# kevslinger/DTQN

Measured on AMD Instinct MI355X. Metric: env-steps/sec + TD-updates/sec, DiscreteCarFlag-v0 ctx=50 b=32, 1/2/4/8 GPU, higher is better.
Workload: dtype f32; 1 GPU; DiscreteCarFlag-v0 shapes (BASELINE config 1): ctx=50, d_model=64, 8 heads, 2 layers, obs 3 f32, 3 actions, batch 32 per GPU, history 50, device replay 2500 x 200 steps; global_batch=32, parallelism=dp1, sampler=device

## Files before the change

### dtqn_amd/csrc/dtqn_api.cpp

```cpp
#include <hip/hip_runtime.h>

#include <cstdlib>

#include "dtqn_hip.h"
#include "dtqn_limits.h"

extern "C" const char* dtqn_build_info(void) {
#ifdef DTQN_BUILD_INFO
    return DTQN_BUILD_INFO;
#else
    return "dtqn_hip (unstamped build)";
#endif
}

static void* g_profile_buffer = nullptr;
extern "C" int dtqn_debug_set_profile_buffer(void* dev_buffer) {
    g_profile_buffer = dev_buffer;
    return DTQN_OK;
}
extern "C" void* dtqn_debug_profile_buffer(void) { return g_profile_buffer; }

static int policy_cus() {
    int dev = 0, n = 0;
    if (hipGetDevice(&dev) != hipSuccess || hipDeviceGetAttribute(&n, hipDeviceAttributeMultiprocessorCount, dev) != hipSuccess || n <= 0) return 256;
    return n;
}
extern "C" int dtqn_td_row_split(const DtqnNet* net, int batch) {
    if (!net || batch < 1) return 1;
    const int cus = policy_cus();
    const char* e = getenv("DTQN_ROW_SPLIT");
    if (e != nullptr && e[0] == '0') return 1;
    const bool covered = !net->tiled && net->lp == 64 && !net->identity &&
                         (net->d_model == 64 || (net->d_model == 128 && net->gate == DTQN_GATE_RES));
    if (!covered) return 1;
    if (e != nullptr && e[0] == '1') return 2;
    if (e != nullptr && e[0] == '4') return 4;
    if (3 * batch * 2 <= cus) return 4;
    if (net->d_model == 64) {
        if (batch * 4 <= cus) return 4;
        if (batch * 2 <= cus) return 2;
    }
    return 1;
}
extern "C" int dtqn_td_latency_mode(const DtqnNet* net, int batch) {
    if (dtqn_td_row_split(net, batch) < 2) return 0;
    const char* e = getenv("DTQN_ROW_SPLIT");
    if (e != nullptr && (e[0] == '1' || e[0] == '4')) return 1;
    return 3 * batch * 2 <= policy_cus() ? 1 : 0;
}
extern "C" int dtqn_td_prefers_tiled(const DtqnNet* net, int batch) {
    if (!net || batch < 1 || net->tiled) return 0;
    if (dtqn_ws_lite(net->tiled, net->d_model, net->head_dim, net->d_real))
        return dtqn_td_row_split(net, batch) == 4 && dtqn_td_latency_mode(net, batch) ? 0 : 1;
    const bool covered = net->d_model == 128 && net->gate == DTQN_GATE_RES && !net->identity && net->lp == 64 && net->dropout == 0.f &&
                         net->bag_size == 0;
    if (!covered) return 0;
    const char* e = getenv("DTQN_TRAIN_TILED");
    if (e != nullptr) return atoi(e) != 0 ? 1 : 0;
    return dtqn_td_row_split(net, batch) == 1 ? 1 : 0;
}
extern "C" int dtqn_td_xch_floats(const DtqnNet* net, int batch) {
    if (!net || batch < 1) return 0;
    return 3 * batch * net->num_layers * (3 * net->lp / 4) * 2 * net->d_model;
}
extern "C" int dtqn_td_xch_flags(const DtqnNet* net, int batch) {
    if (!net || batch < 1) return 0;
    return 3 * batch * net->num_layers * 6 + 16;
}

extern "C" int dtqn_td_update(const DtqnNet* net, const DtqnReplay* rp, const DtqnTd* td, void* stream) {
    int rc;
    if ((rc = dtqn_td_forward(net, rp, td, stream)) != DTQN_OK) return rc;
    if ((rc = dtqn_td_backward(net, rp, td, stream)) != DTQN_OK) return rc;
    if ((rc = dtqn_td_wgrad(net, td, stream)) != DTQN_OK) return rc;
    if ((rc = dtqn_td_reduce(net, td, stream)) != DTQN_OK) return rc;
    return dtqn_td_clip_adam(net, td, stream);
}

extern "C" int dtqn_td_gradients_pipelined(const DtqnNet* net, const DtqnReplay* rp, const DtqnTd* td, const DtqnTd* td_next, int have_target,
                                           int draw_step, void* stream) {
    int rc;
    if (draw_step < 0) return DTQN_ERR_ARG;
    if ((rc = dtqn_td_forward_part(net, rp, td, 0, 2, 4, draw_step, stream)) != DTQN_OK) return rc;
    if (!have_target && (rc = dtqn_td_forward_part(net, rp, td, 2, 1, 4, draw_step, stream)) != DTQN_OK) return rc;
    rc = td_next != nullptr ? dtqn_td_backward_ahead(net, rp, td, td_next, draw_step + 1, stream) : dtqn_td_backward(net, rp, td, stream);
    if (rc != DTQN_OK) return rc;
    if ((rc = dtqn_td_wgrad(net, td, stream)) != DTQN_OK) return rc;
    return dtqn_td_reduce(net, td, stream);
}
extern "C" int dtqn_td_update_pipelined(const DtqnNet* net, const DtqnReplay* rp, const DtqnTd* td, const DtqnTd* td_next, int have_target,
                                        int draw_step, void* stream) {
    const int rc = dtqn_td_gradients_pipelined(net, rp, td, td_next, have_target, draw_step, stream);
    return rc != DTQN_OK ? rc : dtqn_td_clip_adam(net, td, stream);
}

namespace dtqn {
int forward_infer(const DtqnNet* net, const float* theta, const float* obs, const uint8_t* actions, int batch, int n,
                  float* q_out, float* q_last_host, void* stream, float* xch, int32_t* xflags, const int32_t* last_rows, int in_rows,
                  uint32_t drop_seed, uint32_t drop_step, int train_mode);
int tiled_forward_actor(const DtqnNet* net, const float* theta, const float* obs, const uint8_t* actions, int batch, int n, int in_rows,
                        float* q_out, float* workspace, int train_mode, uint32_t drop_seed, uint32_t drop_step, hipStream_t stream, const int32_t* lens = nullptr);
}
extern "C" int dtqn_forward_tiled_strided(const DtqnNet* net, const float* theta, const float* obs, const uint8_t* actions,
                                          int batch, int n, int in_rows, float* q_out, float* workspace, void* stream);

extern "C" int dtqn_replay_push(const DtqnReplay* rp, const DtqnReplayRecord* recs_host, const float* obs_host, int n,
                                void* stream) {
    if (!rp || n < 0) return DTQN_ERR_ARG;
    if (n == 0) return DTQN_OK;
    if (!recs_host || !obs_host) return DTQN_ERR_ARG;
    return dtqn_replay_apply(rp, recs_host, obs_host, n, stream);
}

extern "C" int dtqn_actor_forward(const DtqnNet* net, const float* theta, const void* ctx_host, void* ctx_dev, int n,
                                  float* q_dev, float* q_last_host, float* workspace, int train_mode, uint32_t dropout_seed,
                                  uint32_t dropout_step, void* stream) {
    if (!net || !theta || !ctx_host || !ctx_dev || !q_dev || !q_last_host) return DTQN_ERR_ARG;
    if (n < 1 || n > net->ctx_len) return DTQN_ERR_ARG;
    hipStream_t s = (hipStream_t)stream;
    const size_t obs_bytes = sizeof(float) * (size_t)net->ctx_len * net->obs_dim;
    if (hipMemcpyAsync(ctx_dev, ctx_host, obs_bytes + (size_t)net->ctx_len, hipMemcpyHostToDevice, s) != hipSuccess) return DTQN_ERR_LAUNCH;
    const float* obs = static_cast<const float*>(ctx_dev);
    const uint8_t* actions = static_cast<const uint8_t*>(ctx_dev) + obs_bytes;
    if (!net->tiled) {
        const bool split = workspace != nullptr && n > net->lp / 2 && dtqn_td_row_split(net, 1) >= 2;
        float* xch = split ? workspace : nullptr;
        int32_t* xflags = split ? reinterpret_cast<int32_t*>(workspace + dtqn_td_xch_floats(net, 1)) : nullptr;
        return dtqn::forward_infer(net, theta, obs, actions, 1, n, q_dev, q_last_host, stream, xch, xflags, nullptr, 0, dropout_seed, dropout_step, train_mode);
    }
    const int rc = dtqn::tiled_forward_actor(net, theta, obs, actions, 1, n, n, q_dev, workspace, train_mode, dropout_seed, dropout_step, s);
    if (rc != DTQN_OK) return rc;
    if (hipMemcpyAsync(q_last_host, q_dev + (size_t)(n - 1) * net->num_actions, sizeof(float) * net->num_actions,
                       hipMemcpyDeviceToHost, s) != hipSuccess)
        return DTQN_ERR_LAUNCH;
    return DTQN_OK;
}

extern "C" int dtqn_actor_forward_batch(const DtqnNet* net, const float* theta, const void* ctx_host, void* ctx_dev, int n_envs,
                                        int n_max, float* q_dev, float* q_last_host, float* workspace, int train_mode,
                                        uint32_t dropout_seed, uint32_t dropout_step, void* stream) {
    if (!net || !theta || !ctx_host || !ctx_dev || !q_dev || !q_last_host || n_envs < 1) return DTQN_ERR_ARG;
    if (n_max < 1 || n_max > net->ctx_len) return DTQN_ERR_ARG;
    hipStream_t s = (hipStream_t)stream;
    const int L = net->ctx_len;
    const size_t obs_bytes = sizeof(float) * (size_t)n_envs * L * net->obs_dim;
    const size_t act_bytes = (((size_t)n_envs * L) + 3) & ~(size_t)3;
    const size_t total = obs_bytes + act_bytes + sizeof(int32_t) * (size_t)n_envs;
    const int32_t* lens_h = reinterpret_cast<const int32_t*>(static_cast<const uint8_t*>(ctx_host) + obs_bytes + act_bytes);
    for (int i = 0; i < n_envs; ++i)
        if (lens_h[i] < 1 || lens_h[i] > n_max) return DTQN_ERR_ARG;
    if (hipMemcpyAsync(ctx_dev, ctx_host, total, hipMemcpyHostToDevice, s) != hipSuccess) return DTQN_ERR_LAUNCH;
    const float* obs = static_cast<const float*>(ctx_dev);
    const uint8_t* actions = static_cast<const uint8_t*>(ctx_dev) + obs_bytes;
    const int32_t* lens = reinterpret_cast<const int32_t*>(static_cast<const uint8_t*>(ctx_dev) + obs_bytes + act_bytes);
    if (net->tiled) {
        const int rc = dtqn::tiled_forward_actor(net, theta, obs, actions, n_envs, n_max, L, q_dev, workspace, train_mode, dropout_seed,
                                                 dropout_step, (hipStream_t)stream, lens);
        if (rc != DTQN_OK) return rc;
        for (int i = 0; i < n_envs; ++i)
            if (hipMemcpyAsync(q_last_host + (size_t)i * net->num_actions, q_dev + ((size_t)i * n_max + (lens_h[i] - 1)) * net->num_actions,
                               sizeof(float) * net->num_actions, hipMemcpyDeviceToHost, s) != hipSuccess)
                return DTQN_ERR_LAUNCH;
        return DTQN_OK;
    }
    const bool split = workspace != nullptr && n_max > net->lp / 2 && dtqn_td_row_split(net, n_envs) >= 2;
    float* xch = split ? workspace : nullptr;
    int32_t* xflags = split ? reinterpret_cast<int32_t*>(workspace + dtqn_td_xch_floats(net, n_envs)) : nullptr;
    return dtqn::forward_infer(net, theta, obs, actions, n_envs, n_max, q_dev, q_last_host, stream, xch, xflags, lens, L, dropout_seed, dropout_step, train_mode);
}

extern "C" int dtqn_forward_train(const DtqnNet* net, const float* theta, const float* obs, const uint8_t* actions, const float* bag_obs,
                                  const uint8_t* bag_actions, int batch, int n, float* q_out, float* workspace, void* stream) {
    return dtqn_forward_train_drop(net, theta, obs, actions, bag_obs, bag_actions, batch, n, q_out, workspace, 0u, -1, stream);
}
extern "C" int dtqn_backward_dq(const DtqnNet* net, const float* theta, const float* obs, const uint8_t* actions, const float* bag_obs,
                                const uint8_t* bag_actions, int batch, int n, const float* dq, float* workspace, float* grad, float* dobs,
                                void* stream) {
    return dtqn_backward_dq_drop(net, theta, obs, actions, bag_obs, bag_actions, batch, n, dq, workspace, grad, dobs, 0u, -1, stream);
}
```

### dtqn_amd/csrc/dtqn_backward.hip

```cpp
#include "dtqn_device.hpp"
#include "dtqn_bwd_device.hpp"
#include "dtqn_gru.hpp"
#include "dtqn_wgrad_direct.hpp"
#include "dtqn_forward_body.hpp"

#ifndef DTQN_SPLIT_ATTN_MFMA
#define DTQN_SPLIT_ATTN_MFMA 1
#endif
#ifndef DTQN_BWD_DOX
#define DTQN_BWD_DOX 1
#endif
#ifndef DTQN_BWD_DOX_EARLY_FLAG
#define DTQN_BWD_DOX_EARLY_FLAG 1
#endif
#ifndef DTQN_BWD_FOLD_GUARD
#define DTQN_BWD_FOLD_GUARD 0
#endif
#if DTQN_BWD_FOLD_GUARD
#define DTQN_BWD_GUARD(w, q) Own::valid_fast(w, q)
#else
#define DTQN_BWD_GUARD(w, q) Own::valid(w, q)
#endif

namespace dtqn {

struct BwdArgs {
    DtqnNet net;
    const float* theta;
    const float* act;
    float* grd;
    float* small;
    const float* q3;
    float* stats_partial;
    const float* obs;
    const uint8_t* actions;
    const float* rewards;
    const uint8_t* dones;
    long long obs_ep_stride, act_ep_stride, rew_ep_stride;
    const int32_t* ep_idx;
    const int32_t* start;
    int batch, history;
    float gamma;
    long long* prof;
    float* xch;
    int32_t* xflags;
    uint32_t drop_thresh, drop_seed;
    float drop_scale;
    const int32_t* step_counter;
    FuseArgs fuse;
};

template <bool AHEAD> struct AheadArgs {};
template <> struct AheadArgs<true> { FwdArgs f; };

template <int D, int MT, int HD, int NW, bool GRU, int RS, bool DROP, bool FUSE = false, bool AHEAD = false, bool PAD = false>
__global__ __launch_bounds__(NW * 64) void dtqn_backward_kernel(BwdArgs a, AheadArgs<AHEAD> ahead) {
    static_assert(RS == 1 || RS == 2 || RS == 4, "one, two or four row slices");
    static_assert(!PAD || (RS == 4 && MT == 1 && !GRU && !DROP && !FUSE && D == 64), "width padding rides with the four-slice residual-gate chain");
    if constexpr (AHEAD) {
        static_assert(RS == 4 && MT == 1 && !GRU && !DROP && !FUSE && D <= 64, "the target pass ahead rides with the four-slice residual-gate chain");
        if ((int)blockIdx.x >= a.batch * RS) {
            forward_body_wl<D, 1, HD, NW, 4, false, PAD>(ahead.f);
            return;
        }
    }
    constexpr int NT = NW * 64;
    constexpr int LP = MT * 16;
    constexpr int LPF = LP * RS;
    constexpr int LDX = D + 4;
    constexpr int GW = D >= 64 ? 64 : D;
    constexpr int NG = D / GW;
    constexpr int NC = D >= 128 ? D / 2 : 2 * D;
    constexpr bool OST = D <= 64;
    constexpr int W5C = ((OST ? 6 : 5) * GW > NC ? (OST ? 6 : 5) * GW : NC);
    constexpr int LD5 = W5C + 4;
    constexpr int MGX = pick_mg(D / 16, MT, NW);
    using Own = Owned<D, MT, MGX, NW>;
    const DtqnNet& net = a.net;
    const Thr t = make_thr();
    const Thr& t_outer = t;
    if constexpr (FUSE) {
        if ((int)blockIdx.x >= a.batch * RS) {
            const DirectCtx ctx{a.act, a.grd, a.small, a.fuse.grad, a.batch, RS, a.fuse.n_small};
            fuse_role<NW>(net, a.fuse, ctx, (int)blockIdx.x - a.batch * RS, reinterpret_cast<float*>(dtqn_smem), t);
            return;
        }
    }
    int b, pos;
    slice_block_map((int)blockIdx.x, a.batch, RS, b, pos);
    const int slice = RS - 1 - pos;
    const int R0 = slice * LP;
    const int Lfull = net.ctx_len, A = net.num_actions, AP = net.ap, H = net.num_heads, adim = net.action_dim;
    const int L = Lfull - R0 < LP ? Lfull - R0 : LP;
    const bool ident = RS > 1 ? false : net.identity != 0;
    const int dreal = PAD ? net.d_real : D;
    constexpr bool gru = GRU;
    const float* __restrict__ theta = a.theta;
    const float* rec = a.act + (size_t)b * net.act_stride;
    float* grec = a.grd + (size_t)b * net.grd_stride;
    float* srec = a.small + ((size_t)b * RS + slice) * net.sp_stride;
    auto rf = [&](const float* base, int off, int w) -> const float* { return base + off + (size_t)R0 * w; };
    auto gf = [&](float* base, int off, int w) -> float* { return base + off + (size_t)R0 * w; };
    auto mf = [&](const float* base, int off, int ctiles) -> const float* { return base + off + (size_t)(R0 / 16) * ctiles * 8; };
    const DtqnRsrc grs = DTQN_XCH_RSRC(grec, (size_t)net.grd_stride * 4);
    constexpr bool WT = FUSE || (kOptBwdWT && !(GRU && !DROP && MT >= 2 && NW == 8));
    auto g_store4 = [&](float* p, float4 v) {
        if constexpr (WT) dtqn_xch_store4(grs, (int)(p - grec) * 4, v);
        else st4(p, v);
    };
    auto g_tile_store = [&](const float* s_, int ld_, float* g_, int rows, int cols, int gld = 0) {
        if constexpr (WT) {
            const int c4 = cols >> 2;
            if (gld == 0) gld = cols;
            const int base = (int)(g_ - grec);
            for (int idx = t_outer.tid; idx < rows * c4; idx += NT) {
                const int r = idx / c4, c = (idx - r * c4) * 4;
                dtqn_xch_store4(grs, (base + r * gld + c) * 4, ld4(s_ + r * ld_ + c));
            }
        } else {
            tile_store<NW>(s_, ld_, g_, rows, cols, t_outer, gld);
        }
    };
    auto s_store = [&](float* p, float v) {
        if constexpr (FUSE) DTQN_AGENT_STORE(p, v);
        else *p = v;
    };

    float* DX = reinterpret_cast<float*>(dtqn_smem);
    float* T2 = DX + LP * LDX;
    float* W5 = T2 + LP * LDX;
    float* dq_s = W5 + LPF * LD5;
    float* delta_s = dq_s + LP * AP;
    float* lse_s = delta_s + (GW / HD) * LPF;
    float* red = lse_s + (GW / HD) * LPF;
    constexpr int PARTS = NT / D >= 1 ? NT / D : 1;
    float* st_s = red + PARTS * 2 * D;
    float* DU = st_s + 4 * LP;

    const int ep = a.ep_idx[b], st0 = a.start[b] + R0;
    Drop dr = drop_off();
    if constexpr (DROP) dr = Drop{a.drop_thresh, a.drop_scale, a.drop_seed, (uint32_t)a.step_counter[1], (uint32_t)b};
    int ps = 0;
    DTQN_PROF(a.prof, ps++);
    static_assert(HD <= 16 || (HD == 32 && RS == 4 && MT == 1), "delta-in-epilogue: a head inside one 16-column tile, or two tiles wide on the four-slice chain");
    constexpr bool SPLITS = kOptSplitS && MT == 1 && 2 * (D / 16) == NW && 2 * (GW / 16) == NW;
    std::conditional_t<SPLITS, StageDyWSplit<D, NW, D / 16>, StageDyW<D, MT, pick_mg(D / 16, MT, NW), NW, D / 16>> g_h1;
    g_h1.prefetch(theta + net.off_head1_w, D, t);
    TileRegs<NW, LP, D> tr;
    TileRegs<NW, LP, D> trh;
    trh.load(rf(rec, net.ao_hh, D), D, t);
    if (!ident) tr.load(rf(rec, net.ao_layer0 + (net.num_layers - 1) * net.act_layer_stride + net.al_s2, D), D, t);

    static_assert(4 * LP <= NT, "one statistics value per thread");
    auto st_fetch = [&](int l) -> float {
        const float* lr = rec + net.ao_layer0 + (size_t)l * net.act_layer_stride;
        if (t.tid >= 4 * LP) return 0.f;
        return t.tid < 2 * LP ? rf(lr, net.al_st1, 2)[t.tid] : rf(lr, net.al_st2, 2)[t.tid - 2 * LP];
    };
    float st_next = st_fetch(net.num_layers - 1);

    {
        const float* q0 = a.q3 + (((size_t)0 * a.batch + b) * LPF + R0) * AP;
        const float* q1 = a.q3 + (((size_t)1 * a.batch + b) * LPF + R0) * AP;
        const float* q2 = a.q3 + (((size_t)2 * a.batch + b) * LPF + R0) * AP;
        const float inv_count = 1.0f / ((float)a.batch * (float)a.history);
        DTQN_PROF(a.prof, 24);
        for (int idx = t.tid; idx < LP * AP; idx += NT) dq_s[idx] = 0.f;
        __syncthreads();
        DTQN_PROF(a.prof, 25);
        if (t.wave == 0)
            td_loss_wave(q0, q1, q2, AP, A, Lfull - R0, LP, a.history, a.gamma, inv_count,
                         a.actions + (size_t)ep * a.act_ep_stride + st0, a.rewards + (size_t)ep * a.rew_ep_stride + st0,
                         a.dones + (size_t)ep * a.rew_ep_stride + st0, dq_s, a.stats_partial + ((size_t)b * RS + slice) * 8, t.lane);
        DTQN_PROF(a.prof, 26);
        __syncthreads();
        DTQN_PROF(a.prof, 27);
        if constexpr (WT) {
            for (int idx = t.tid; idx < LP * AP / 4; idx += NT) g_store4(gf(grec, net.go_dq, AP) + 4 * idx, ld4(dq_s + 4 * idx));
        } else {
            for (int idx = t.tid; idx < LP * AP; idx += NT) gf(grec, net.go_dq, AP)[idx] = dq_s[idx];
        }
    }

    DTQN_PROF(a.prof, ps++);
    {
        const float* __restrict__ W2 = theta + net.off_head2_w;
        constexpr int C4 = D / 4;
#pragma unroll
        for (int k4 = 0; k4 < TileRegs<NW, LP, D>::N; ++k4) {
            const int idx4 = t.tid + k4 * NT;
            if (idx4 < LP * C4) {
                const int r = idx4 / C4, c0 = (idx4 - r * C4) * 4;
                const float hv[4] = {trh.v[k4].x, trh.v[k4].y, trh.v[k4].z, trh.v[k4].w};
                float g4[4];
#pragma unroll
                for (int e = 0; e < 4; ++e) {
                    float g = 0.f;
                    if (hv[e] > 0.f)
                        for (int c = 0; c < A; ++c) g = fmaf(dq_s[r * AP + c], W2[c * D + c0 + e], g);
                    g4[e] = g;
                }
                st4(T2 + r * LDX + c0, make_float4(g4[0], g4[1], g4[2], g4[3]));
            }
        }
    }
    __syncthreads();
    g_h1.retire();
    g_tile_store(T2, LDX, gf(grec, net.go_dhh, D), LP, D);
    if constexpr (SPLITS) g_h1.run(T2, LDX, t, red, [&](int r, int c, float v) { DX[r * LDX + c] = v; });
    else g_h1.run(T2, LDX, t, [&](int r, int c, float v) { DX[r * LDX + c] = v; });
    __syncthreads();
    DTQN_PROF(a.prof, ps++);

    for (int l = net.num_layers - 1; l >= 0; --l) {
        Thr t = t_outer;
#define DTQN_RELAUNDER() do { if constexpr (D >= 128 && MT >= 4) { DTQN_ASM_KEEP(t.tid); DTQN_ASM_KEEP(t.lane); DTQN_ASM_KEEP(t.wave); DTQN_ASM_KEEP(t.i); DTQN_ASM_KEEP(t.kq); } \
        else if constexpr (D == 64 && MT >= 2 && NW <= 8 && (RS == 1 || (GRU && RS == 2))) { int tid_ = (int)threadIdx.x; DTQN_ASM_KEEP(tid_); t.tid = tid_; t.lane = tid_ & 63; t.wave = tid_ >> 6; t.i = t.lane & 15; t.kq = t.lane >> 4; } } while (0)
        DTQN_RELAUNDER();
        const float* __restrict__ th = layer_theta(net, theta, l);
        const float* lrec = rec + net.ao_layer0 + (size_t)l * net.act_layer_stride;
        float* lgrd = grec + net.go_layer0 + (size_t)l * net.grd_layer_stride;
        float* lsm = srec + net.so_ln + l * 4 * D;
        const float* __restrict__ W1 = th + net.lo_f1_w;
        const float* __restrict__ W2 = th + net.lo_f2_w;
        StageDyW<D, MT, pick_mg(NC / 16, MT, NW), NW, NC / 16> g_dh;
        g_dh.prefetch(W2, 4 * D, t);
        if (t.tid < 4 * LP) st_s[t.tid] = st_next;
        if (l > 0) st_next = st_fetch(l - 1);

        if (!ident) {
            if (l == net.num_layers - 1) DTQN_PROF(a.prof, 28);
            tr.to_lds(T2, LDX, t);
            if (l == net.num_layers - 1) DTQN_PROF(a.prof, 29);
            __syncthreads();
            if (l == net.num_layers - 1) DTQN_PROF(a.prof, 30);
            layernorm_backward<D, NW, FUSE, PAD>(DX, T2, DX, false, LDX, LP, st_s + 2 * LP, th + net.lo_ln2_w, lsm + 2 * D, red, t, false, dreal);
            if (l == net.num_layers - 1) DTQN_PROF(a.prof, 31);
            __syncthreads();
        }
        DTQN_PROF(a.prof, ps++);
        tr.load(rf(lrec, net.al_s1, D), D, t);
        if (gru) {
            gru_gate_backward<D, MT, NW>(DX, T2, LDX, W5, LD5, theta + net.off_gate_mlp, net, lrec + net.al_gate2, lgrd + net.gl_gate2, t, LPF, R0);
            __syncthreads();
        }
        {
            const float* m2 = mf(lrec, net.al_m2, D / 16);
            for (int idx = t.tid; idx < LP * D; idx += NT) {
                const int r = idx / D, c = idx - r * D;
                const float dy = gru ? T2[r * LDX + c] : DX[r * LDX + c];
                T2[r * LDX + c] = mask_bit(m2, D / 16, r, c) ? drop_apply(dr, DROP_FFN, l, (uint32_t)((R0 + r) * D + c), dy) : 0.f;
            }
        }
        __syncthreads();
        DTQN_RELAUNDER();
        {
            f32x4 xacc[Own::PER_WAVE][MGX];
#pragma unroll
            for (int q = 0; q < Own::PER_WAVE; ++q)
#pragma unroll
                for (int m = 0; m < MGX; ++m) xacc[q][m] = zero4();
            float w1f[2][NC / 4];
            constexpr bool SPLITK = kOptSplitK && Own::ITEMS * 2 == NW && Own::PER_WAVE == 1 && MGX == 1 && NC % 32 == 0;
            constexpr bool HALFW = kOptHalfW && !SPLITK && NC % 32 == 0;
            const int sk_it = t.wave % Own::ITEMS, sk_kh = t.wave / Own::ITEMS;
            const unsigned long long* mh = reinterpret_cast<const unsigned long long*>(mf(lrec, net.al_mh, 4 * D / 16));
            constexpr int MGH = pick_mg(NC / 16, MT, NW);
#pragma clang loop unroll_count(D >= 128 ? 1 : 4)
            for (int c0 = 0; c0 < 4 * D; c0 += NC) {
                g_dh.retire();
                if (c0 == 0) g_tile_store(T2, LDX, gf(lgrd, net.gl_df, D), LP, D);
                unsigned long long mw[MGH][4];
                g_dh.run(T2, LDX, t,
                         [&](int kt, int mg) {
#pragma unroll
                             for (int m = 0; m < MGH; ++m)
#pragma unroll
                                 for (int r = 0; r < 4; ++r)
                                     mw[m][r] = mh[((mg * MGH + m) * (4 * D / 16) + (c0 >> 4) + kt) * 4 + r];
                         },
                         [&](int r, int c, float v) {
                             const unsigned long long w = mw[(r >> 4) % MGH][r & 3];
                             W5[r * LD5 + c] = ((w >> t.lane) & 1ull) ? v : 0.f;
                         });
                if constexpr (SPLITK) {
                    float (&wh)[NC / 8] = *reinterpret_cast<float (*)[NC / 8]>(&w1f[0][0]);
                    frag_dyw_fetch<NC / 2>(wh, W1 + (size_t)(c0 + sk_kh * (NC / 2)) * D + sk_it * 16 + t.i, D, t);
                } else if constexpr (HALFW) {
                    float (&wh)[NC / 8] = *reinterpret_cast<float (*)[NC / 8]>(&w1f[0][0]);
                    if (DTQN_BWD_GUARD(t.wave, 0)) frag_dyw_fetch<NC / 2>(wh, W1 + (size_t)c0 * D + Own::nt(t.wave, 0) * 16 + t.i, D, t);
                } else if (DTQN_BWD_GUARD(t.wave, 0))
                    frag_dyw_fetch<NC>(w1f[0], W1 + (size_t)c0 * D + Own::nt(t.wave, 0) * 16 + t.i, D, t);
                if constexpr (FUSE) {
                    if (c0 == 0 && l + 1 < net.num_layers) DTQN_WAIT_VMEM();
                }
                __syncthreads();
                if constexpr (FUSE) {
                    if (c0 == 0 && l + 1 < net.num_layers) fuse_arrive(a.fuse.counters, net.num_layers - 2 - l, t);
                }
                if (SPLITK || DTQN_BWD_GUARD(t.wave, 0)) {
#pragma unroll
                    for (int q = 0; q < (SPLITK || HALFW ? NC / 8 : NC / 4); ++q) DTQN_ASM_KEEP(w1f[0][q]);
                }
                g_tile_store(W5, LD5, gf(lgrd, net.gl_dhp, 4 * D) + c0, LP, NC, 4 * D);
                if constexpr (SPLITK) {
                    const float (&wh)[NC / 8] = *reinterpret_cast<const float (*)[NC / 8]>(&w1f[0][0]);
                    frag_dyw_mma<NC / 2, 1>(W5 + sk_kh * (NC / 2), LD5, wh, t, xacc[0]);
                } else if constexpr (HALFW) {
                    float (&wa)[NC / 8] = *reinterpret_cast<float (*)[NC / 8]>(&w1f[0][0]);
                    float (&wb)[NC / 8] = *reinterpret_cast<float (*)[NC / 8]>(&w1f[1][0]);
#pragma unroll
                    for (int q = 0; q < Own::PER_WAVE; ++q) {
                        const float* wcol = W1 + (size_t)c0 * D + Own::nt(t.wave, q) * 16 + t.i;
                        const float* rows = W5 + Own::mg(t.wave, q) * MGX * 16 * LD5;
                        if (DTQN_BWD_GUARD(t.wave, q)) {
                            frag_dyw_fetch<NC / 2>(wb, wcol + (size_t)(NC / 2) * D, D, t);
                            frag_dyw_mma<NC / 2, MGX>(rows, LD5, wa, t, xacc[q]);
                        }
                        if (q + 1 < Own::PER_WAVE && DTQN_BWD_GUARD(t.wave, q + 1))
                            frag_dyw_fetch<NC / 2>(wa, W1 + (size_t)c0 * D + Own::nt(t.wave, q + 1) * 16 + t.i, D, t);
                        if (DTQN_BWD_GUARD(t.wave, q)) frag_dyw_mma<NC / 2, MGX>(rows + NC / 2, LD5, wb, t, xacc[q]);
                    }
                } else {
#pragma unroll
                    for (int q = 0; q < Own::PER_WAVE; ++q) {
                        if (q + 1 < Own::PER_WAVE && DTQN_BWD_GUARD(t.wave, q + 1))
                            frag_dyw_fetch<NC>(w1f[(q + 1) & 1], W1 + (size_t)c0 * D + Own::nt(t.wave, q + 1) * 16 + t.i, D, t);
                        if (DTQN_BWD_GUARD(t.wave, q))
                            frag_dyw_mma<NC, MGX>(W5 + Own::mg(t.wave, q) * MGX * 16 * LD5, LD5, w1f[q & 1], t, xacc[q]);
                    }
                }
                if (c0 + NC < 4 * D) g_dh.prefetch(W2 + c0 + NC, 4 * D, t);
                __syncthreads();
            }
            if constexpr (SPLITK) {
                if (t.wave >= Own::ITEMS) {
#pragma unroll
                    for (int r4 = 0; r4 < 4; ++r4) W5[((t.wave - Own::ITEMS) * 4 + r4) * 64 + t.lane] = xacc[0][0][r4];
                }
                __syncthreads();
                if (t.wave < Own::ITEMS) {
#pragma unroll
                    for (int r4 = 0; r4 < 4; ++r4) xacc[0][0][r4] += W5[(t.wave * 4 + r4) * 64 + t.lane];
                }
            }
            float* dst = ident ? DU : DX;
#pragma unroll
            for (int q = 0; q < Own::PER_WAVE; ++q) {
                if (DTQN_BWD_GUARD(t.wave, q)) {
                    const int c = Own::nt(t.wave, q) * 16 + t.i;
#pragma unroll
                    for (int m = 0; m < MGX; ++m)
#pragma unroll
                        for (int r4 = 0; r4 < 4; ++r4) {
                            const int r = (Own::mg(t.wave, q) * MGX + m) * 16 + t.kq * 4 + r4;
                            if (ident) dst[r * LDX + c] = xacc[q][m][r4];
                            else dst[r * LDX + c] += xacc[q][m][r4];
                        }
                }
            }
        }
        tr.to_lds(T2, LDX, t);
        constexpr bool DOX = RS > 1 && DTQN_BWD_DOX && DTQN_SPLIT_ATTN_MFMA;
        TileRegs<NW, LP, GW> tq, to, tk[RS], tv[RS], tqu[DOX ? RS : 1];
        constexpr int NLSE = (GW / HD) * LPF, LSE_N = (NLSE + NT - 1) / NT;
        float lse_r[LSE_N];
        auto load_group = [&](int g) {
            if constexpr (kOptLse) {
#pragma unroll
                for (int k = 0; k < LSE_N; ++k) {
                    const int idx = t.tid + k * NT;
                    lse_r[k] = lrec[net.al_lse + g * NLSE + (idx < NLSE ? idx : 0)];
                }
            }
            const float* qkv0 = lrec + net.al_qkv + g * GW;
            tq.load(qkv0 + (size_t)R0 * 3 * D, 3 * D, t);
            if constexpr (DOX) {
#pragma unroll
                for (int j = 1; j < RS; ++j)
                    if (j > slice) tqu[j].load(qkv0 + (size_t)j * LP * 3 * D, 3 * D, t);
            }
#pragma unroll
            for (int j = 0; j < RS; ++j)
                if (j <= slice) {
                    tk[j].load(qkv0 + (size_t)j * LP * 3 * D + D, 3 * D, t);
                    tv[j].load(qkv0 + (size_t)j * LP * 3 * D + 2 * D, 3 * D, t);
                }
            if (OST) to.load(rf(lrec, net.al_o, D) + g * GW, D, t);
        };
        load_group(0);
        const float* __restrict__ Wo = th + net.lo_out_w;
        const float* __restrict__ Win = th + net.lo_in_w;
        std::conditional_t<SPLITS, StageDyWSplit<D, NW, GW / 16>, StageDyW<D, MT, pick_mg(GW / 16, MT, NW), NW, GW / 16>> g_do;
        g_do.prefetch(Wo, D, t);
        __syncthreads();
        DTQN_PROF(a.prof, ps++);
        if (!ident)
            layernorm_backward<D, NW, FUSE, PAD>(DX, T2, DX, false, LDX, LP, st_s, th + net.lo_ln1_w, lsm, red, t, false, dreal);
        else
            layernorm_backward<D, NW, FUSE, PAD>(DU, T2, DX, true, LDX, LP, st_s + 2 * LP, th + net.lo_ln2_w, lsm + 2 * D, red, t, false, dreal);
        __syncthreads();
        DTQN_PROF(a.prof, ps++);
        if (gru) {
            gru_gate_backward<D, MT, NW>(DX, T2, LDX, W5, LD5, theta + net.off_gate_attn, net, lrec + net.al_gate1, lgrd + net.gl_gate1, t, LPF, R0);
            __syncthreads();
        }
        {
            const float* m1 = mf(lrec, net.al_m1, D / 16);
            for (int idx = t.tid; idx < LP * D; idx += NT) {
                const int r = idx / D, c = idx - r * D;
                const float dy = gru ? T2[r * LDX + c] : DX[r * LDX + c];
                T2[r * LDX + c] = mask_bit(m1, D / 16, r, c) ? dy : 0.f;
            }
        }
        DTQN_RELAUNDER();
        {
            f32x4 xacc[Own::PER_WAVE][MGX];
#pragma unroll
            for (int q = 0; q < Own::PER_WAVE; ++q)
#pragma unroll
                for (int m = 0; m < MGX; ++m) xacc[q][m] = zero4();
            float winf[2][GW / 4];
            constexpr bool SPLITW = kOptSplitW && Own::ITEMS * 2 == NW && Own::PER_WAVE == 1 && MGX == 1 && GW % 32 == 0;
            constexpr int WPC = GW / 2;
            const int sw_it = t.wave % Own::ITEMS, sw_kh = t.wave / Own::ITEMS;
            float wpc[2][WPC / 4];
            auto piece_fetch = [&](float (&wf)[WPC / 4], int g_, int j) {
                const int u = sw_kh * 3 + j, part = u >> 1, off = (u & 1) * WPC;
                frag_dyw_fetch<WPC>(wf, Win + (size_t)(part * D + g_ * GW + off) * D + sw_it * 16 + t.i, D, t);
            };
            const float* o_g = rf(lrec, net.al_o, D);
            float* W5r = W5 + R0 * LD5;
            constexpr int MGO = pick_mg(GW / 16, MT, NW);
#pragma unroll
            for (int g = 0; g < NG; ++g) {
                tq.to_lds(W5r, LD5, t);
                if constexpr (DOX) {
#pragma unroll
                    for (int j = 1; j < RS; ++j)
                        if (j > slice) tqu[j].to_lds(W5 + j * LP * LD5, LD5, t);
                }
#pragma unroll
                for (int j = 0; j < RS; ++j)
                    if (j <= slice) {
                        tk[j].to_lds(W5 + j * LP * LD5 + GW, LD5, t);
                        tv[j].to_lds(W5 + j * LP * LD5 + 2 * GW, LD5, t);
                    }
                if (OST) to.to_lds(W5r + 5 * GW, LD5, t);
                if constexpr (kOptLse) {
#pragma unroll
                    for (int k = 0; k < LSE_N; ++k) {
                        const int idx = t.tid + k * NT;
                        if (idx < NLSE) lse_s[idx] = lse_r[k];
                    }
                } else {
                    for (int idx = t.tid; idx < NLSE; idx += NT) lse_s[idx] = lrec[net.al_lse + g * NLSE + idx];
                }
                if constexpr (HD > 16) {
                    for (int idx = t.tid; idx < (GW / HD) * LP; idx += NT) delta_s[(idx / LP) * LPF + R0 + idx % LP] = 0.f;
                }
                __syncthreads();
                g_do.retire();
                if (g == 0 && !DOX) g_tile_store(T2, LDX, gf(lgrd, net.gl_da, D), LP, D);
                float ov[MGO][4];
                auto do_pre = [&](int kt, int mg) {
                    if (!OST) {
#pragma unroll
                        for (int m = 0; m < MGO; ++m)
#pragma unroll
                            for (int r = 0; r < 4; ++r)
                                ov[m][r] = o_g[(size_t)((mg * MGO + m) * 16 + t.kq * 4 + r) * D + g * GW + kt * 16 + t.i];
                    }
                };
                auto do_epi = [&](int r, int c, float v) {
                    W5r[r * LD5 + 3 * GW + c] = v;
                    float p = v * (OST ? W5r[r * LD5 + 5 * GW + c] : ov[(r >> 4) % MGO][r & 3]);
#pragma unroll
                    for (int m = 1; m < (HD < 16 ? HD : 16); m <<= 1) p += __shfl_xor(p, m);
                    if constexpr (HD <= 16) {
                        if ((t.i & (HD - 1)) == 0) delta_s[(c / HD) * LPF + R0 + r] = p;
                    } else {
                        if (t.i == 0) atomicAdd(&delta_s[(c / HD) * LPF + R0 + r], p);
                    }
                };
                if constexpr (SPLITS) g_do.run(T2, LDX, t, red, do_pre, do_epi);
                else g_do.run(T2, LDX, t, do_pre, do_epi);
                if constexpr (SPLITW) piece_fetch(wpc[0], g, 0);
                else if (DTQN_BWD_GUARD(t.wave, 0))
                    frag_dyw_fetch<GW>(winf[0], Win + (size_t)(0 * D + g * GW) * D + Own::nt(t.wave, 0) * 16 + t.i, D, t);
                __syncthreads();
                DTQN_PROF(a.prof, ps++);
                if constexpr (DOX) {
                    constexpr int PAIRS = RS * (RS - 1) / 2, SEG = LP * GW + (GW / HD) * LP;
                    const size_t grp = ((size_t)b * net.num_layers + l) * NG + g;
                    float* xg = a.xch + grp * PAIRS * LP * 2 * GW;
                    int32_t* fg = a.xflags + grp * PAIRS;
                    auto pair_id = [](int s_, int r_) { return s_ * (s_ - 1) / 2 + r_; };
                    static_assert((RS - 1) * SEG <= PAIRS * LP * 2 * GW, "dO segments fit the exchange region");
                    if (slice > 0) {
                        const DtqnRsrc rs = DTQN_XCH_RSRC(xg + (size_t)(slice - 1) * SEG, SEG * 4);
                        constexpr int C4 = GW / 4;
                        for (int idx = t.tid; idx < LP * C4; idx += NT) {
                            const int r = idx / C4, c = (idx - r * C4) * 4;
                            dtqn_xch_store4(rs, idx * 16, ld4(W5r + r * LD5 + 3 * GW + c));
                        }
                        for (int idx = t.tid; idx < (GW / HD) * LP / 4; idx += NT) {
                            const int h = idx / (LP / 4), r4 = (idx - h * (LP / 4)) * 4;
                            dtqn_xch_store4(rs, (LP * GW + h * LP + r4) * 4, ld4(delta_s + h * LPF + R0 + r4));
                        }
#if DTQN_BWD_DOX_EARLY_FLAG
                        DTQN_WAIT_VMEM();
                        __syncthreads();
                        if (t.tid < slice) DTQN_AGENT_STORE(fg + pair_id(slice, t.tid), (int32_t)1);
#endif
                    }
                    auto between = [&]() {
#if !DTQN_BWD_DOX_EARLY_FLAG
                        if (slice > 0) {
                            DTQN_WAIT_VMEM();
                            __syncthreads();
                            if (t.tid < slice) DTQN_AGENT_STORE(fg + pair_id(slice, t.tid), (int32_t)1);
                        }
#endif
                        const int nsnd = RS - 1 - slice;
                        if (nsnd > 0) {
                            if (t.tid < nsnd)
                                while (DTQN_AGENT_LOAD(fg + pair_id(slice + 1 + t.tid, slice)) == 0) DTQN_SPIN_PAUSE();
                            __syncthreads();
                            constexpr int C4 = GW / 4, TILE4 = LP * C4, DEL4 = (GW / HD) * LP / 4, SEG4 = TILE4 + DEL4;
                            const DtqnRsrc rs = DTQN_XCH_RSRC(xg + (size_t)slice * SEG, nsnd * SEG * 4);
                            for (int idx = t.tid; idx < nsnd * SEG4; idx += NT) {
                                const int k = idx / SEG4, e = idx - k * SEG4, sndr = slice + 1 + k;
                                const float4 v = dtqn_xch_load4(rs, (k * SEG + e * 4) * 4);
                                if (e < TILE4) {
                                    const int r = e / C4, c = (e - r * C4) * 4;
                                    st4(W5 + (sndr * LP + r) * LD5 + 3 * GW + c, v);
                                } else {
                                    const int d = e - TILE4, h = d / (LP / 4), r4 = (d - h * (LP / 4)) * 4;
                                    st4(delta_s + h * LPF + sndr * LP + r4, v);
                                }
                            }
                            __syncthreads();
                            if (t.tid < nsnd) DTQN_AGENT_STORE(fg + pair_id(slice + 1 + t.tid, slice), (int32_t)0);
                        }
                    };
                    if constexpr (PAD)
                        attention_backward_group_mfma<HD, NW>(W5, LD5, GW, LP, Lfull, delta_s, lse_s, t, nullptr, 0, R0, LPF, dr, l, g * (GW / HD),
                                                              true, LPF / 16, between, (float)net.hd_real);
                    else
                    attention_backward_group_mfma<HD, NW>(W5, LD5, GW, LP, Lfull, delta_s, lse_s, t, nullptr, 0, R0, LPF, dr, l, g * (GW / HD),
                                                          true, LPF / 16, between);
                    __syncthreads();
                } else {
                attention_backward_group<HD, NW, (HD >= kAttnMfmaMinHeadDim) || (RS > 1 && DTQN_SPLIT_ATTN_MFMA)>(W5, LD5, GW, LP, Lfull, delta_s, lse_s, t, nullptr, 0, R0, LPF, dr, l, g * (GW / HD));
                __syncthreads();
                if (RS > 1) {
                    constexpr int PAIRS = RS * (RS - 1) / 2;
                    const size_t grp = ((size_t)b * net.num_layers + l) * NG + g;
                    float* xg = a.xch + grp * PAIRS * LP * 2 * GW;
                    int32_t* fg = a.xflags + grp * PAIRS;
                    auto pair_id = [](int s_, int r_) { return s_ * (s_ - 1) / 2 + r_; };
                    if (slice > 0) {
                        const DtqnRsrc rs = DTQN_XCH_RSRC(xg + (size_t)pair_id(slice, 0) * LP * 2 * GW, R0 * 2 * GW * 4);
                        constexpr int C4 = 2 * GW / 4;
                        for (int idx = t.tid; idx < R0 * C4; idx += NT) {
                            const int r = idx / C4, c = (idx - r * C4) * 4;
                            dtqn_xch_store4(rs, idx * 16, ld4(W5 + r * LD5 + GW + c));
                        }
                        DTQN_WAIT_VMEM();
                        __syncthreads();
                        if (t.tid < slice) DTQN_AGENT_STORE(fg + pair_id(slice, t.tid), (int32_t)1);
                    }
                    for (int sndr = slice + 1; sndr < RS; ++sndr)
                        xch_recv<NW, true>(W5r + GW, LD5, xg + (size_t)pair_id(sndr, slice) * LP * 2 * GW, LP, 2 * GW,
                                           fg + pair_id(sndr, slice), t);
                }
                }
                DTQN_PROF(a.prof, ps++);
                if constexpr (SPLITW) {
#pragma unroll
                    for (int q = 0; q < WPC / 4; ++q) DTQN_ASM_KEEP(wpc[0][q]);
                } else if (DTQN_BWD_GUARD(t.wave, 0)) {
#pragma unroll
                    for (int q = 0; q < GW / 4; ++q) DTQN_ASM_KEEP(winf[0][q]);
                }
                if (g == 0 && DOX) g_tile_store(T2, LDX, gf(lgrd, net.gl_da, D), LP, D);
                for (int idx = t.tid; idx < LP * 3 * (GW / 4); idx += NT) {
                    const int r = idx / (3 * (GW / 4)), rem = idx - r * (3 * (GW / 4));
                    const int which = rem / (GW / 4), c = (rem - which * (GW / 4)) * 4;
                    const float* sp = W5r + r * LD5 + (which == 0 ? 4 * GW : which * GW) + c;
                    g_store4(gf(lgrd, net.gl_dqkv, 3 * D) + (size_t)r * 3 * D + which * D + g * GW + c, ld4(sp));
                }
                if constexpr (SPLITW) {
#pragma unroll
                    for (int j = 0; j < 3; ++j) {
                        if (j + 1 < 3) piece_fetch(wpc[(j + 1) & 1], g, j + 1);
                        const int u = sw_kh * 3 + j, part = u >> 1, off = (u & 1) * WPC;
                        frag_dyw_mma<WPC, 1>(W5r + (part == 0 ? 4 * GW : part * GW) + off, LD5, wpc[j & 1], t, xacc[0]);
                    }
                } else
#pragma unroll
                for (int q = 0; q < Own::PER_WAVE; ++q) {
#pragma unroll
                    for (int part = 0; part < 3; ++part) {
                        const int step = q * 3 + part;
                        const int nq = part < 2 ? q : q + 1, np = part < 2 ? part + 1 : 0;
                        if (nq < Own::PER_WAVE && DTQN_BWD_GUARD(t.wave, nq))
                            frag_dyw_fetch<GW>(winf[(step + 1) & 1], Win + (size_t)(np * D + g * GW) * D + Own::nt(t.wave, nq) * 16 + t.i, D, t);
                        if (DTQN_BWD_GUARD(t.wave, q)) {
                            const float* rows = W5r + Own::mg(t.wave, q) * MGX * 16 * LD5 + (part == 0 ? 4 * GW : part * GW);
                            frag_dyw_mma<GW, MGX>(rows, LD5, winf[step & 1], t, xacc[q]);
                        }
                    }
                }
                if (g + 1 < NG) {
                    g_do.prefetch(Wo + (g + 1) * GW, D, t);
                    load_group(g + 1);
                }
                __syncthreads();
            }
            if (!ident) {
                if (l > 0) tr.load(rf(rec, net.ao_layer0 + (l - 1) * net.act_layer_stride + net.al_s2, D), D, t);
            } else {
                tr.load(l == 0 ? rf(rec, net.ao_x0, D) : rf(rec, net.ao_layer0 + (l - 1) * net.act_layer_stride + net.al_s2, D), D, t);
            }
            if constexpr (SPLITW) {
                if (t.wave >= Own::ITEMS) {
#pragma unroll
                    for (int r4 = 0; r4 < 4; ++r4) W5[((t.wave - Own::ITEMS) * 4 + r4) * 64 + t.lane] = xacc[0][0][r4];
                }
                __syncthreads();
                if (t.wave < Own::ITEMS) {
#pragma unroll
                    for (int r4 = 0; r4 < 4; ++r4) xacc[0][0][r4] += W5[(t.wave * 4 + r4) * 64 + t.lane];
                }
            }
            float* dst = ident ? DU : DX;
#pragma unroll
            for (int q = 0; q < Own::PER_WAVE; ++q) {
                if (DTQN_BWD_GUARD(t.wave, q)) {
                    const int c = Own::nt(t.wave, q) * 16 + t.i;
#pragma unroll
                    for (int m = 0; m < MGX; ++m)
#pragma unroll
                        for (int r4 = 0; r4 < 4; ++r4) {
                            const int r = (Own::mg(t.wave, q) * MGX + m) * 16 + t.kq * 4 + r4;
                            if (ident) dst[r * LDX + c] = xacc[q][m][r4];
                            else dst[r * LDX + c] += xacc[q][m][r4];
                        }
                }
            }
        }
        __syncthreads();
        DTQN_PROF(a.prof, ps++);
        if (ident) {
            tr.to_lds(T2, LDX, t);
            __syncthreads();
            layernorm_backward<D, NW, FUSE, PAD>(DU, T2, DX, true, LDX, LP, st_s, th + net.lo_ln1_w, lsm, red, t, false, dreal);
            __syncthreads();
        }
    }

    DTQN_PROF(a.prof, ps++);
    if (dr.thresh != 0u) {
        for (int idx = t.tid; idx < LP * D; idx += NT) {
            const int r = idx / D, c = idx - r * D;
            DX[r * LDX + c] = drop_apply(dr, DROP_EMB, 0, (uint32_t)((R0 + r) * D + c), DX[r * LDX + c]);
        }
        __syncthreads();
    }
    g_tile_store(DX, LDX, gf(grec, net.go_dx0, D), LP, D);
    const float* obs_rows = a.obs + (size_t)ep * a.obs_ep_stride + (size_t)st0 * net.obs_dim;
    const uint8_t* act_rows = a.actions + (size_t)ep * a.act_ep_stride + st0;
    if (net.discrete) {
        const int KE = net.ke, KEP = net.kep, e = net.embed_per_obs, V = net.vocab, O = net.obs_dim;
        const float* __restrict__ We = theta + net.off_obs_w;
        float* dein = W5;
        for (int idx = t.tid; idx < LP * KEP; idx += NT) {
            const int r = idx / KEP, k = idx - r * KEP;
            float g = 0.f;
            if (r < L && k < KE)
                for (int d = 0; d < D - adim; ++d) g = fmaf(DX[r * LDX + adim + d], We[(size_t)d * KE + k], g);
            dein[idx] = g;
        }
        __syncthreads();
        for (int idx = t.tid; idx < V * e; idx += NT) {
            const int v = idx / e, c = idx - v * e;
            float g = 0.f;
            for (int r = 0; r < L; ++r)
                for (int j = 0; j < O; ++j) {
                    int tok = (int)obs_rows[(size_t)r * O + j];
                    tok = tok < 0 ? 0 : (tok >= V ? V - 1 : tok);
                    if (tok == v) g += dein[r * KEP + j * e + c];
                }
            s_store(srec + net.so_tab + idx, g);
        }
    }
    if (adim > 0) {
        for (int idx = t.tid; idx < A * adim; idx += NT) {
            const int v = idx / adim, c = idx - v * adim;
            float g = 0.f;
            if (Lfull == 1) {
                if ((int)act_rows[0] == v) g = DX[c];
            } else {
                for (int r = R0 > 0 ? 0 : 1; r < L; ++r)
                    if ((int)act_rows[r - 1] == v) g += DX[r * LDX + c];
            }
            s_store(srec + net.so_act + idx, g);
        }
    }
    if constexpr (FUSE) {
        DTQN_WAIT_VMEM();
        __syncthreads();
        fuse_arrive(a.fuse.counters, net.num_layers, t);
    }
}

static size_t bwd_lds_bytes(const DtqnNet* net) {
    const int LP = net->lp, D = net->d_model, HD = net->head_dim;
    const int GW = D >= 64 ? 64 : D, NC = D >= 128 ? D : 2 * D;
    const int ntile = D <= 64 ? 6 : 5;
    const int W5C = ntile * GW > NC ? ntile * GW : NC;
    const int NT = waves_for(*net) * 64;
    const int PARTS = NT / D >= 1 ? NT / D : 1;
    size_t fl = 2 * (size_t)LP * (D + 4) + (size_t)LP * (W5C + 4) + (size_t)LP * net->ap + 2 * (size_t)(GW / HD) * LP +
                (size_t)PARTS * 2 * D + 4 * (size_t)LP;
    if (net->identity) fl += (size_t)LP * (D + 4);
    return fl * sizeof(float);
}

template <int D, int MT, int HD, int NW, bool GRU, int RS, bool DROP, bool FUSE = false>
static int launch_bwd3(const BwdArgs& a, hipStream_t stream) {
    const size_t lds = bwd_lds_bytes(&a.net);
    static size_t attr_lds[kMaxDevices] = {};
    raise_lds_limit(reinterpret_cast<const void*>(&dtqn_backward_kernel<D, MT, HD, NW, GRU, RS, DROP, FUSE>), lds, attr_lds);
    (void)hipGetLastError();
    const int grid = a.batch * RS + (FUSE ? a.fuse.n_role : 0);
    hipLaunchKernelGGL((dtqn_backward_kernel<D, MT, HD, NW, GRU, RS, DROP, FUSE>), dim3(grid), dim3(NW * 64), lds, stream, a, AheadArgs<false>{});
    return hipGetLastError() == hipSuccess ? DTQN_OK : DTQN_ERR_LAUNCH;
}
template <int HD, bool PAD = false>
static int launch_bwd_ahead(const BwdArgs& a, const FwdArgs& f, hipStream_t stream) {
    const size_t lb = bwd_lds_bytes(&a.net), lf = fwd_lds_bytes(&a.net, true);
    const size_t lds = lb > lf ? lb : lf;
    if (lds > 160 * 1024) return DTQN_ERR_CONFIG;
    static size_t attr_lds[kMaxDevices] = {};
    raise_lds_limit(reinterpret_cast<const void*>(&dtqn_backward_kernel<64, 1, HD, 8, false, 4, false, false, true, PAD>), lds, attr_lds);
    (void)hipGetLastError();
    AheadArgs<true> ah;
    ah.f = f;
    ah.f.block0 = a.batch * 4;
    hipLaunchKernelGGL((dtqn_backward_kernel<64, 1, HD, 8, false, 4, false, false, true, PAD>), dim3(a.batch * 4 + f.batch * 4), dim3(8 * 64), lds, stream, a, ah);
    return hipGetLastError() == hipSuccess ? DTQN_OK : DTQN_ERR_LAUNCH;
}
template <int HD, bool PAD>
static int launch_bwd_lite(const BwdArgs& a, hipStream_t stream) {
    const size_t lds = bwd_lds_bytes(&a.net);
    static size_t attr_lds[kMaxDevices] = {};
    raise_lds_limit(reinterpret_cast<const void*>(&dtqn_backward_kernel<64, 1, HD, 8, false, 4, false, false, false, PAD>), lds, attr_lds);
    (void)hipGetLastError();
    hipLaunchKernelGGL((dtqn_backward_kernel<64, 1, HD, 8, false, 4, false, false, false, PAD>), dim3(a.batch * 4), dim3(8 * 64), lds, stream, a, AheadArgs<false>{});
    return hipGetLastError() == hipSuccess ? DTQN_OK : DTQN_ERR_LAUNCH;
}
template <int D, int MT, int HD, int NW, bool GRU, int RS>
static int launch_bwd2(const BwdArgs& a, hipStream_t stream) {
    if constexpr (RS == 4 && !GRU && NW == kFuseWaves) {
        if (a.fuse.n_role > 0) {
            if (bwd_lds_bytes(&a.net) < (kFuseWaves + (size_t)(kDSmallFused / 64) * kFuseWaves * 64) * sizeof(float) ||
                bwd_lds_bytes(&a.net) < direct_lds_floats(kFuseWaves) * sizeof(float)) return DTQN_ERR_CONFIG;
            if (a.drop_thresh != 0u) return launch_bwd3<D, MT, HD, NW, GRU, RS, true, true>(a, stream);
            return launch_bwd3<D, MT, HD, NW, GRU, RS, false, true>(a, stream);
        }
    }
    if (a.fuse.n_role > 0) return DTQN_ERR_CONFIG;
    if (a.drop_thresh != 0u) return launch_bwd3<D, MT, HD, NW, GRU, RS, true>(a, stream);
    return launch_bwd3<D, MT, HD, NW, GRU, RS, false>(a, stream);
}
template <int D, int MT, int HD, int NW>
static int launch_bwd(const BwdArgs& a, hipStream_t stream) {
    if (a.net.gate == DTQN_GATE_GRU) {
        if constexpr (D <= 64) return launch_bwd2<D, MT, HD, NW, true, 1>(a, stream);
        else return DTQN_ERR_CONFIG;
    }
    return launch_bwd2<D, MT, HD, NW, false, 1>(a, stream);
}

}

using namespace dtqn;

extern "C" int dtqn_lds_bytes_backward(const DtqnNet* net) {
    if (!net) return 0;
    const size_t b = bwd_lds_bytes(net);
    return b <= 160 * 1024 ? (int)b : 0;
}

extern "C" int dtqn_td_wgrad_is_fused(const DtqnNet* net, const DtqnTd* td) {
    FuseArgs f;
    return fuse_plan(net, td, &f) ? 1 : 0;
}

static int td_backward(const DtqnNet* net, const DtqnReplay* rp, const DtqnTd* td, const DtqnTd* td_next, int draw_step_next, void* stream);

extern "C" int dtqn_td_backward(const DtqnNet* net, const DtqnReplay* rp, const DtqnTd* td, void* stream) {
    return td_backward(net, rp, td, nullptr, -1, stream);
}

extern "C" int dtqn_td_backward_ahead(const DtqnNet* net, const DtqnReplay* rp, const DtqnTd* td, const DtqnTd* td_next, int draw_step_next,
                                      void* stream) {
    if (!td_next || draw_step_next < 0) return DTQN_ERR_ARG;
    return td_backward(net, rp, td, td_next, draw_step_next, stream);
}

static int td_backward(const DtqnNet* net, const DtqnReplay* rp, const DtqnTd* td, const DtqnTd* td_next, int draw_step_next, void* stream) {
    if (!net || !rp || !td || td->batch < 1) return DTQN_ERR_ARG;
    if (td->history < 1 || td->history > net->ctx_len) return DTQN_ERR_ARG;
    if (net->tiled) return td_next ? DTQN_ERR_CONFIG : tiled_td_backward(net, rp, td, (hipStream_t)stream);
    if (bwd_lds_bytes(net) > 160 * 1024) return DTQN_ERR_CONFIG;
    BwdArgs a;
    a.net = *net;
    a.theta = td->theta_pol;
    a.act = td->act; a.grd = td->grd; a.small = td->small; a.q3 = td->q3; a.stats_partial = td->stats_partial;
    a.obs = rp->obs; a.actions = rp->actions; a.rewards = rp->rewards; a.dones = rp->dones;
    a.obs_ep_stride = (long long)(rp->max_steps + 1) * rp->obs_dim;
    a.act_ep_stride = rp->max_steps + 1;
    a.rew_ep_stride = rp->max_steps;
    a.ep_idx = td->ep_idx; a.start = td->start;
    a.batch = td->batch; a.history = td->history; a.gamma = td->gamma;
    a.prof = dtqn_debug_profile_buffer() ? static_cast<long long*>(dtqn_debug_profile_buffer()) + 64 : nullptr;
    a.xch = td->xch; a.xflags = td->xflags;
    a.drop_thresh = net->dropout > 0.f ? (uint32_t)((double)net->dropout * 4294967296.0) : 0u;
    a.drop_scale = net->dropout > 0.f ? 1.0f / (1.0f - net->dropout) : 1.0f;
    a.drop_seed = td->dropout_seed; a.step_counter = td->step_counter;
    fuse_plan(net, td, &a.fuse);
    const int D = net->d_model, MT = net->lp / 16, HD = net->head_dim, NW = waves_for(*net);
    hipStream_t s = (hipStream_t)stream;
    if (dtqn_ws_lite(net->tiled, D, HD, net->d_real)) {
        if (td->row_split != 4 || net->lp != 64 || net->identity || net->gate != DTQN_GATE_RES || !a.xch || !a.xflags || a.drop_thresh != 0u ||
            a.fuse.n_role > 0 || NW != 8) return DTQN_ERR_CONFIG;
        const bool pad = net->d_real > 0;
        if (td_next != nullptr) {
            if (!dtqn_td_fwd_slices4_ok(net) || !td_next->sample_in_kernel || td_next->batch != td->batch || !td_next->xch || !td_next->xflags ||
                !td_next->q3) return DTQN_ERR_CONFIG;
            FwdArgs f;
            td_forward_args(net, rp, td_next, 2, draw_step_next, &f);
            f.nseq = td_next->batch;
            f.prof = nullptr;
            if (HD == 8 && pad) return launch_bwd_ahead<8, true>(a, f, s);
            if (HD == 16 && pad) return launch_bwd_ahead<16, true>(a, f, s);
            if (HD == 32) return pad ? launch_bwd_ahead<32, true>(a, f, s) : launch_bwd_ahead<32, false>(a, f, s);
            return DTQN_ERR_CONFIG;
        }
        if (HD == 8 && pad) return launch_bwd_lite<8, true>(a, s);
        if (HD == 16 && pad) return launch_bwd_lite<16, true>(a, s);
        if (HD == 32) return pad ? launch_bwd_lite<32, true>(a, s) : launch_bwd_lite<32, false>(a, s);
        return DTQN_ERR_CONFIG;
    }
    if (td->row_split == 2 || td->row_split == 4) {
        if (net->lp != 64 || net->identity || !a.xch || !a.xflags) return DTQN_ERR_CONFIG;
        if (net->gate == DTQN_GATE_GRU) {
            if (td->row_split == 4) {
                if (D == 64 && HD == 8) return launch_bwd2<64, 1, 8, 8, true, 4>(a, s);
                if (D == 64 && HD == 16) return launch_bwd2<64, 1, 16, 8, true, 4>(a, s);
                return DTQN_ERR_CONFIG;
            }
            if (D == 64 && HD == 8) return launch_bwd2<64, 2, 8, 8, true, 2>(a, s);
            if (D == 64 && HD == 16) return launch_bwd2<64, 2, 16, 8, true, 2>(a, s);
            return DTQN_ERR_CONFIG;
        }
        if (td_next != nullptr) {
            if (td->row_split != 4 || net->gate != DTQN_GATE_RES || a.drop_thresh != 0u || a.fuse.n_role > 0 || !dtqn_td_fwd_slices4_ok(net) ||
                !td_next->sample_in_kernel || td_next->batch != td->batch || !td_next->xch || !td_next->xflags || !td_next->q3 || NW != 8)
                return DTQN_ERR_CONFIG;
            FwdArgs f;
            td_forward_args(net, rp, td_next, 2, draw_step_next, &f);
            f.nseq = td_next->batch;
            f.prof = nullptr;
            if (D == 64 && HD == 8) return launch_bwd_ahead<8>(a, f, s);
            if (D == 64 && HD == 16) return launch_bwd_ahead<16>(a, f, s);
            return DTQN_ERR_CONFIG;
        }
        if (td->row_split == 4) {
            if (D == 64 && HD == 8) return launch_bwd2<64, 1, 8, 8, false, 4>(a, s);
            if (D == 64 && HD == 16) return launch_bwd2<64, 1, 16, 8, false, 4>(a, s);
            if (D == 128 && HD == 16) return launch_bwd2<128, 1, 16, 8, false, 4>(a, s);
            return DTQN_ERR_CONFIG;
        }
        if (D == 64 && HD == 8) return launch_bwd2<64, 2, 8, 8, false, 2>(a, s);
        if (D == 64 && HD == 16) return launch_bwd2<64, 2, 16, 8, false, 2>(a, s);
        if (D == 128 && HD == 16) return launch_bwd2<128, 2, 16, 8, false, 2>(a, s);
        return DTQN_ERR_CONFIG;
    }
#define DTQN_BWD_CASE(d, mt, hd, nw) \
    if (D == d && MT == mt && HD == hd && NW == nw) return launch_bwd<d, mt, hd, nw>(a, s);
    DTQN_WS_TRAIN_INSTANCES(DTQN_BWD_CASE)
#undef DTQN_BWD_CASE
    return DTQN_ERR_CONFIG;
}
```

### dtqn_amd/csrc/dtqn_gfx950.hpp

```cpp
#pragma once
#include <hip/hip_runtime.h>

struct LanePair {
    float v[2];
    __device__ __forceinline__ float operator[](int k) const { return v[k]; }
};
__device__ __forceinline__ LanePair dtqn_lane_swap32(float x) {
    const unsigned u = __float_as_uint(x);
    const auto r = __builtin_amdgcn_permlane32_swap(u, u, false, false);
    return LanePair{{__uint_as_float(r[0]), __uint_as_float(r[1])}};
}
__device__ __forceinline__ LanePair dtqn_lane_swap16(float x) {
    const unsigned u = __float_as_uint(x);
    const auto r = __builtin_amdgcn_permlane16_swap(u, u, false, false);
    return LanePair{{__uint_as_float(r[0]), __uint_as_float(r[1])}};
}
#define DTQN_LANE_SWAP32(x) dtqn_lane_swap32(x)
#define DTQN_LANE_SWAP16(x) dtqn_lane_swap16(x)
#define DTQN_AGENT_LOAD(p) __hip_atomic_load(p, __ATOMIC_RELAXED, __HIP_MEMORY_SCOPE_AGENT)
#define DTQN_AGENT_STORE(p, v) __hip_atomic_store(p, v, __ATOMIC_RELAXED, __HIP_MEMORY_SCOPE_AGENT)
#define DTQN_SYSTEM_LOAD(p) __hip_atomic_load(p, __ATOMIC_RELAXED, __HIP_MEMORY_SCOPE_SYSTEM)
#define DTQN_SYSTEM_STORE(p, v) __hip_atomic_store(p, v, __ATOMIC_RELAXED, __HIP_MEMORY_SCOPE_SYSTEM)
#define DTQN_AGENT_ADD(p, v) __hip_atomic_fetch_add(p, v, __ATOMIC_RELAXED, __HIP_MEMORY_SCOPE_AGENT)
#define DTQN_SPIN_PAUSE() __builtin_amdgcn_s_sleep(2)
#define DTQN_SPIN_PAUSE_LONG() __builtin_amdgcn_s_sleep(12)
#define DTQN_WAIT_VMEM() asm volatile("s_waitcnt vmcnt(0)" ::: "memory")
#define DTQN_SCHED_FENCE() __builtin_amdgcn_sched_barrier(0)
typedef unsigned dtqn_u32x4 __attribute__((ext_vector_type(4)));
typedef __amdgpu_buffer_rsrc_t DtqnRsrc;
#define DTQN_XCH_RSRC(ptr, bytes) __builtin_amdgcn_make_buffer_rsrc((void*)(ptr), 0, (int)(bytes), 0x00020000)
__device__ __forceinline__ void dtqn_xch_store4(DtqnRsrc r, int byte_off, float4 v) {
    dtqn_u32x4 u = {__float_as_uint(v.x), __float_as_uint(v.y), __float_as_uint(v.z), __float_as_uint(v.w)};
    __builtin_amdgcn_raw_buffer_store_b128(u, r, byte_off, 0, 16);
}
__device__ __forceinline__ float4 dtqn_xch_load4(DtqnRsrc r, int byte_off) {
    const dtqn_u32x4 u = __builtin_amdgcn_raw_buffer_load_b128(r, byte_off, 0, 16);
    return make_float4(__uint_as_float(u[0]), __uint_as_float(u[1]), __uint_as_float(u[2]), __uint_as_float(u[3]));
}
__device__ __forceinline__ void dtqn_xch_store1(DtqnRsrc r, int byte_off, float v) {
    __builtin_amdgcn_raw_buffer_store_b32(__float_as_uint(v), r, byte_off, 0, 16);
}
__device__ __forceinline__ float dtqn_xch_load1(DtqnRsrc r, int byte_off) {
    return __uint_as_float(__builtin_amdgcn_raw_buffer_load_b32(r, byte_off, 0, 16));
}
#define DTQN_ROW_ROR(x, n) __uint_as_float(__builtin_amdgcn_mov_dpp(__float_as_uint(x), 0x120 + (n), 0xf, 0xf, true))
#define DTQN_EXP2(x) __builtin_amdgcn_exp2f(x)
#define DTQN_ASM_KEEP(x) asm volatile("" : "+v"(x))
```

### dtqn_amd/csrc/dtqn_wgrad.hip

```cpp
#include <mutex>
#include "dtqn_device.hpp"
#include "dtqn_wgrad_direct.hpp"

namespace dtqn {

constexpr int kMaxWJobs = 48;
struct WgradArgs {
    DtqnNet net;
    DtqnWJob jobs[kMaxWJobs];
    const float* act;
    const float* grd;
    float* gsplit;
    const float* small;
    int batch, n_split, n_jobs;
    int n_small;
    int row_split;
    int small_blocks;
    int xcd_map;
    int n_wtiles;
};

__device__ __forceinline__ void small_partials_block(const WgradArgs& a, int sb, int split) {
    const DtqnNet& net = a.net;
    const int D = net.d_model;
    const int n_ln = net.num_layers * 4 * D;
    const int n_tab = net.discrete ? net.vocab * net.embed_per_obs : 0;
    const int n_act = net.action_dim > 0 ? net.num_actions * net.action_dim : 0;
    const int b_lo = (int)((long long)a.batch * split / a.n_split);
    const int b_hi = (int)((long long)a.batch * (split + 1) / a.n_split);
    float* out = a.gsplit + (size_t)split * net.n_trainable;
    for (int e = sb * 1024 + (int)threadIdx.x; e < min(a.n_small, (sb + 1) * 1024); e += DTQN_THREADS) {
        int dst, src;
        const float* base = a.small;
        size_t stride = (size_t)net.sp_stride;
        if (e < n_ln) {
            const int l = e / (4 * D);
            dst = net.off_layer0 + l * net.layer_stride + (e - l * 4 * D);
            src = net.so_ln + e;
        } else if (e < n_ln + n_tab) {
            dst = net.off_obs_tab + (e - n_ln);
            src = net.so_tab + (e - n_ln);
        } else if (e < n_ln + n_tab + n_act) {
            dst = net.off_act_emb + (e - n_ln - n_tab);
            src = net.so_act + (e - n_ln - n_tab);
        } else {
            dst = net.off_pos + (e - n_ln - n_tab - n_act);
            src = net.go_dx0 + (e - n_ln - n_tab - n_act);
            base = a.grd;
            stride = (size_t)net.grd_stride;
        }
        float v = 0.f;
        const int per = base == a.small ? a.row_split * net.sp_parts : 1;
        for (int b = b_lo * per; b < b_hi * per; ++b) v += base[(size_t)b * stride + src];
        out[dst] = v;
    }
}

__global__ __launch_bounds__(DTQN_THREADS, 2) void dtqn_wgrad_kernel(WgradArgs a) {
    const Thr t = make_thr();
    const DtqnNet& net = a.net;
    const int LP = net.lp;
    const int P = a.n_wtiles * a.n_split, per = (P + 7) / 8, tile_blocks = per * 8, id = (int)blockIdx.x;
    if (id >= tile_blocks) {
        small_partials_block(a, (id - tile_blocks) % a.small_blocks, (id - tile_blocks) / a.small_blocks);
        return;
    }
    const int pair = a.xcd_map ? (id % 8) * per + id / 8 : id;
    if (pair >= P) return;
    const int split = pair / a.n_wtiles, tile = pair - split * a.n_wtiles;
    int j = 0;
    for (int k = 1; k < a.n_jobs; ++k)
        if (a.jobs[k].tile0 <= tile) j = k;
    const DtqnWJob& job = a.jobs[j];
    const int local = tile - job.tile0;
    const int bn = local / job.tiles_k, bk = local - bn * job.tiles_k;
    const int nbase = bn * 64, kbase = bk * 64;
    const float* xbase = (job.x_in_act ? a.act : a.grd) + job.x_off;
    const size_t xstride = job.x_in_act ? (size_t)net.act_stride : (size_t)net.grd_stride;
    const float* ybase = a.grd + job.dy_off;
    const size_t ystride = (size_t)net.grd_stride;
    const int ycol = nbase + 4 * t.i, xcol = kbase + 4 * t.i;
    const bool yok = ycol < job.ldy, xok = xcol < job.ldx;

    f32x4 acc[4][4];
#pragma unroll
    for (int cn = 0; cn < 4; ++cn)
#pragma unroll
        for (int ck = 0; ck < 4; ++ck) acc[cn][ck] = zero4();
    float4 bsum = make_float4(0.f, 0.f, 0.f, 0.f);

    const int b_lo = (int)((long long)a.batch * split / a.n_split);
    const int b_hi = (int)((long long)a.batch * (split + 1) / a.n_split);
    const bool fast = LP % 16 == 0;
    const int NSUB = fast ? LP / 16 : 4;
    const int steps_per_sub = fast ? 4 : (LP / 4 + NSUB - 1) / NSUB;
    const int units = (b_hi - b_lo) * NSUB * job.n_layers;
    const float4 z4 = make_float4(0.f, 0.f, 0.f, 0.f);
    auto unit_ptrs = [&](int u, const float*& yp, const float*& xp, int& s_lo, int& s_hi) {
        const int lyr = u / ((b_hi - b_lo) * NSUB), ul = u - lyr * (b_hi - b_lo) * NSUB;
        const int b = b_lo + ul / NSUB, sub = ul - (ul / NSUB) * NSUB;
        s_lo = sub * steps_per_sub;
        s_hi = min(LP / 4, s_lo + steps_per_sub);
        yp = ybase + (size_t)b * ystride + (size_t)lyr * job.dy_lstride + (size_t)t.kq * job.ldy + ycol;
        xp = xbase + (size_t)b * xstride + (size_t)lyr * job.x_lstride + (size_t)t.kq * job.ldx + xcol;
    };
    if (fast) {
        float4 av[3][4], bv[3][4];
        auto unit_load = [&](int u, float4 (&a4)[4], float4 (&b4)[4]) {
            const float *yp, *xp;
            int s_lo, s_hi;
            unit_ptrs(u, yp, xp, s_lo, s_hi);
#pragma unroll
            for (int k = 0; k < 4; ++k) {
                a4[k] = yok ? ld4(yp + (size_t)4 * (s_lo + k) * job.ldy) : z4;
                b4[k] = xok ? ld4(xp + (size_t)4 * (s_lo + k) * job.ldx) : z4;
            }
        };
        auto unit_mma = [&](const float4 (&a4)[4], const float4 (&b4)[4]) {
#pragma unroll
            for (int k = 0; k < 4; ++k) {
                bsum.x += a4[k].x; bsum.y += a4[k].y; bsum.z += a4[k].z; bsum.w += a4[k].w;
                const float aa[4] = {a4[k].x, a4[k].y, a4[k].z, a4[k].w};
                const float bb[4] = {b4[k].x, b4[k].y, b4[k].z, b4[k].w};
#pragma unroll
                for (int cn = 0; cn < 4; ++cn)
#pragma unroll
                    for (int ck = 0; ck < 4; ++ck) acc[cn][ck] = mfma16(aa[cn], bb[ck], acc[cn][ck]);
            }
        };
        constexpr int W = DTQN_WAVES;
        int u = t.wave;
        if (u < units) unit_load(u, av[0], bv[0]);
        if (LP <= 64) {
            for (; u < units; u += 2 * W) {
                if (u + W < units) unit_load(u + W, av[1], bv[1]);
                unit_mma(av[0], bv[0]);
                if (u + W < units) {
                    if (u + 2 * W < units) unit_load(u + 2 * W, av[0], bv[0]);
                    unit_mma(av[1], bv[1]);
                }
            }
        } else {
            if (u + W < units) unit_load(u + W, av[1], bv[1]);
            for (; u < units; u += 3 * W) {
                if (u + 2 * W < units) unit_load(u + 2 * W, av[2], bv[2]);
                unit_mma(av[0], bv[0]);
                if (u + W < units) {
                    if (u + 3 * W < units) unit_load(u + 3 * W, av[0], bv[0]);
                    unit_mma(av[1], bv[1]);
                    if (u + 2 * W < units) {
                        if (u + 4 * W < units) unit_load(u + 4 * W, av[1], bv[1]);
                        unit_mma(av[2], bv[2]);
                    }
                }
            }
        }
    }
    for (int u = fast ? units : t.wave; u < units; u += DTQN_WAVES) {
        const float *yp, *xp;
        int s_lo, s_hi;
        unit_ptrs(u, yp, xp, s_lo, s_hi);
        float4 av = (yok && s_lo < s_hi) ? ld4(yp + (size_t)4 * s_lo * job.ldy) : z4;
        float4 bv = (xok && s_lo < s_hi) ? ld4(xp + (size_t)4 * s_lo * job.ldx) : z4;
#pragma unroll 2
        for (int s = s_lo; s < s_hi; ++s) {
            const float4 an = (yok && s + 1 < s_hi) ? ld4(yp + (size_t)4 * (s + 1) * job.ldy) : z4;
            const float4 bn = (xok && s + 1 < s_hi) ? ld4(xp + (size_t)4 * (s + 1) * job.ldx) : z4;
            bsum.x += av.x; bsum.y += av.y; bsum.z += av.z; bsum.w += av.w;
            const float aa[4] = {av.x, av.y, av.z, av.w};
            const float bb[4] = {bv.x, bv.y, bv.z, bv.w};
#pragma unroll
            for (int cn = 0; cn < 4; ++cn)
#pragma unroll
                for (int ck = 0; ck < 4; ++ck) acc[cn][ck] = mfma16(aa[cn], bb[ck], acc[cn][ck]);
            av = an;
            bv = bn;
        }
    }
    bsum.x += __shfl_xor(bsum.x, 16); bsum.y += __shfl_xor(bsum.y, 16); bsum.z += __shfl_xor(bsum.z, 16); bsum.w += __shfl_xor(bsum.w, 16);
    bsum.x += __shfl_xor(bsum.x, 32); bsum.y += __shfl_xor(bsum.y, 32); bsum.z += __shfl_xor(bsum.z, 32); bsum.w += __shfl_xor(bsum.w, 32);

    constexpr int SLD = 68;
    float* slab = reinterpret_cast<float*>(dtqn_smem) + (size_t)t.wave * 65 * SLD;
#pragma unroll
    for (int cn = 0; cn < 4; ++cn)
#pragma unroll
        for (int r = 0; r < 4; ++r)
            st4(slab + (4 * (t.kq * 4 + r) + cn) * SLD + 4 * t.i,
                make_float4(acc[cn][0][r], acc[cn][1][r], acc[cn][2][r], acc[cn][3][r]));
    if (t.kq == 0) st4(slab + 64 * SLD + 4 * t.i, bsum);
    __syncthreads();
    const float* s0 = reinterpret_cast<const float*>(dtqn_smem);
    float* out = a.gsplit + (size_t)split * net.n_trainable;
    for (int idx = t.tid; idx < 64 * 16; idx += DTQN_THREADS) {
        const int nl = idx >> 4, k4 = (idx & 15) * 4;
        const int n = nbase + nl, k = kbase + k4;
        if (n < job.N && k < job.K) {
            float4 v = ld4(s0 + nl * SLD + k4);
#pragma unroll
            for (int wv = 1; wv < DTQN_WAVES; ++wv) {
                const float4 x = ld4(s0 + (size_t)wv * 65 * SLD + nl * SLD + k4);
                v.x += x.x; v.y += x.y; v.z += x.z; v.w += x.w;
            }
            float* op = out + job.w_off + (size_t)n * job.K + k;
            if (k + 3 < job.K && (job.K & 3) == 0) {
                st4(op, v);
            } else {
                const float vv[4] = {v.x, v.y, v.z, v.w};
                for (int c = 0; c < 4; ++c)
                    if (k + c < job.K) op[c] = vv[c];
            }
        }
    }
    if (job.b_off >= 0 && bk == 0 && t.tid < 64) {
        const int n = nbase + t.tid;
        if (n < job.N) {
            float v = 0.f;
#pragma unroll
            for (int wv = 0; wv < DTQN_WAVES; ++wv) v += s0[(size_t)wv * 65 * SLD + 64 * SLD + t.tid];
            out[job.b_off + n] = v;
        }
    }
}

constexpr int kLdsTK = 32, kLdsLDY = 128, kLdsLDX = 160, kLdsThreads = 512;
struct WgradLdsJob {
    DtqnWJob j;
    int tile0;
};
struct WgradLdsArgs {
    DtqnNet net;
    WgradLdsJob jobs[kMaxWJobs];
    const float* act;
    const float* grd;
    float* gsplit;
    int batch, n_split, n_jobs, n_tiles;
};
__global__ __launch_bounds__(kLdsThreads, 2) void dtqn_wgrad_lds_kernel(WgradLdsArgs a) {
    const Thr t = make_thr();
    const DtqnNet& net = a.net;
    const int LP = net.lp;
    float* Ys = reinterpret_cast<float*>(dtqn_smem);
    float* Xs = Ys + kLdsTK * kLdsLDY;
    const int pair = (int)blockIdx.x, split = pair / a.n_tiles, tile = pair - split * a.n_tiles;
    int jx = 0;
    for (int k = 1; k < a.n_jobs; ++k)
        if (a.jobs[k].tile0 <= tile) jx = k;
    const DtqnWJob& job = a.jobs[jx].j;
    const int local = tile - a.jobs[jx].tile0, tk = job.K / 128;
    const int bn = local / tk, bk = local - bn * tk, nbase = bn * 128, kbase = bk * 128;
    const float* xbase = (job.x_in_act ? a.act : a.grd) + job.x_off + kbase;
    const size_t xstride = job.x_in_act ? (size_t)net.act_stride : (size_t)net.grd_stride;
    const float* ybase = a.grd + job.dy_off + nbase;
    const size_t ystride = (size_t)net.grd_stride;
    const int b_lo = (int)((long long)a.batch * split / a.n_split), b_hi = (int)((long long)a.batch * (split + 1) / a.n_split);
    const int live_rows = net.bag_size > 0 ? LP : net.ctx_len;
    const int cps = (live_rows + kLdsTK - 1) / kLdsTK, nb = b_hi - b_lo, nchunks = job.n_layers * nb * cps;
    f32x4 acc[4][2];
#pragma unroll
    for (int cn = 0; cn < 4; ++cn) { acc[cn][0] = zero4(); acc[cn][1] = zero4(); }
    float bsum = 0.f;
    const bool want_bias = job.b_off >= 0 && bk == 0;
    const int sr = t.tid >> 5, sc = (t.tid & 31) * 4;
    float4 yr[2], xr[2];
    auto chunk_load = [&](int c) {
        const int lyr = c / (nb * cps), rem = c - lyr * nb * cps, b = rem / cps, r0 = (rem - b * cps) * kLdsTK;
        const float* yp = ybase + (size_t)(b_lo + b) * ystride + (size_t)lyr * job.dy_lstride + (size_t)r0 * job.ldy + sc;
        const float* xp = xbase + (size_t)(b_lo + b) * xstride + (size_t)lyr * job.x_lstride + (size_t)r0 * job.ldx + sc;
#pragma unroll
        for (int k = 0; k < 2; ++k) {
            yr[k] = ld4(yp + (size_t)(sr + 16 * k) * job.ldy);
            xr[k] = ld4(xp + (size_t)(sr + 16 * k) * job.ldx);
        }
    };
    const int wn = t.wave >> 2, wk = t.wave & 3;
    const float* ya = Ys + t.kq * kLdsLDY + 64 * wn + 4 * t.i;
    const float* xa = Xs + t.kq * kLdsLDX + 32 * wk + 2 * t.i;
    if (nchunks > 0) chunk_load(0);
    for (int c = 0; c < nchunks; ++c) {
        __syncthreads();
#pragma unroll
        for (int k = 0; k < 2; ++k) {
            st4(Ys + (sr + 16 * k) * kLdsLDY + sc, yr[k]);
            st4(Xs + (sr + 16 * k) * kLdsLDX + sc, xr[k]);
        }
        __syncthreads();
        if (c + 1 < nchunks) chunk_load(c + 1);
        const int r0c = (c % cps) * kLdsTK, smax = live_rows - r0c >= kLdsTK ? kLdsTK / 4 : (live_rows - r0c + 3) / 4;
#pragma unroll
        for (int s = 0; s < kLdsTK / 4; ++s) {
            if (s >= smax) break;
            const float4 a4 = ld4(ya + 4 * s * kLdsLDY);
            const float2 b2 = *reinterpret_cast<const float2*>(xa + 4 * s * kLdsLDX);
            const float aa[4] = {a4.x, a4.y, a4.z, a4.w};
#pragma unroll
            for (int cn = 0; cn < 4; ++cn) {
                acc[cn][0] = mfma16(aa[cn], b2.x, acc[cn][0]);
                acc[cn][1] = mfma16(aa[cn], b2.y, acc[cn][1]);
            }
        }
        if (want_bias && t.tid < 128) {
#pragma unroll 8
            for (int r = 0; r < kLdsTK; ++r) bsum += Ys[r * kLdsLDY + t.tid];
        }
    }
    float* out = a.gsplit + (size_t)split * net.n_trainable;
#pragma unroll
    for (int cn = 0; cn < 4; ++cn)
#pragma unroll
        for (int r = 0; r < 4; ++r) {
            const int n = nbase + 64 * wn + 4 * (4 * t.kq + r) + cn, k = kbase + 32 * wk + 2 * t.i;
            *reinterpret_cast<float2*>(out + job.w_off + (size_t)n * job.K + k) = make_float2(acc[cn][0][r], acc[cn][1][r]);
        }
    if (want_bias && t.tid < 128) out[job.b_off + nbase + t.tid] = bsum;
}
static inline bool wgrad_lds_job(const DtqnNet& net, const DtqnWJob& j) {
    return net.tiled && j.N % 128 == 0 && j.K % 128 == 0 && j.ldy % 4 == 0 && j.ldx % 4 == 0;
}
static inline bool wgrad_lds_enabled(const DtqnNet& net) {
    const char* e = getenv("DTQN_WGRAD_LDS");
    return net.tiled && net.d_model % 128 == 0 && net.img_c <= 0 && !(e != nullptr && atoi(e) == 0);
}

struct WgradDirectArgs {
    DtqnNet net;
    DtqnWJob jobs[kMaxWJobs];
    int dtile0[kMaxWJobs];
    const float* act;
    const float* grd;
    float* grad;
    const float* small;
    float* norm_partial;
    int32_t* step_counter;
    int batch, n_jobs, n_small, row_split;
    int n_tiles, n_parts;
    int slots;
    int xcd_tile0[8], xcd_ntiles[8];
    int xcd_map;
    int small_per;
};

__global__ __launch_bounds__(kDirectThreads) void dtqn_wgrad_direct_kernel(WgradDirectArgs a) {
    const Thr t = make_thr();
    const DtqnNet& net = a.net;
    const int tid = t.tid;
    float* red = reinterpret_cast<float*>(dtqn_smem);
    float* slabs = red + kDirectWaves;
    float ss = 0.f;
    const int b = (int)blockIdx.x, tile_blocks = a.slots * 8;
    if (b == 0 && tid == 0) a.step_counter[0] = a.step_counter[1];
    if (b == 0)
        for (int i = (int)gridDim.x + tid; i < a.n_parts; i += kDirectThreads) a.norm_partial[i] = 0.f;
    const int tile = b >= tile_blocks ? a.n_tiles : !a.xcd_map ? b : b / 8 < a.xcd_ntiles[b % 8] ? a.xcd_tile0[b % 8] + b / 8 : a.n_tiles;
    const DirectCtx ctx{a.act, a.grd, a.small, a.grad, a.batch, a.row_split, a.n_small};
    if (b >= tile_blocks) {
        ss = a.small_per == 2 * kDSmall ? direct_small<false, 2 * kDSmall, kDirectWaves>(net, ctx, b - tile_blocks, slabs, t)
                                        : direct_small<false, kDSmall, kDirectWaves>(net, ctx, b - tile_blocks, slabs, t);
    } else if (tile < a.n_tiles) {
        int j = 0;
        for (int k = 1; k < a.n_jobs; ++k)
            if (a.dtile0[k] <= tile) j = k;
        ss = direct_tile<false, kDirectWaves>(net, ctx, a.jobs[j], tile - a.dtile0[j], slabs, t);
    }
    direct_norm_partial<kDirectWaves>(ss, red, a.norm_partial, b, t);
}

static int direct_tiles(const DtqnNet* net, const DtqnWJob* jobs, int* dtile0) {
    int tiles = 0;
    for (int j = 0; j < net->n_wjobs; ++j) {
        if (dtile0) dtile0[j] = tiles;
        tiles += direct_tiles_of(jobs[j]);
    }
    return tiles;
}
struct DirectPlan {
    int dtile0[kMaxWJobs];
    int n_tiles, slots, grid;
    int small_per;
    int grid_max;
    int xcd_tile0[8], xcd_ntiles[8];
};
static DirectPlan direct_plan(const DtqnNet* net, const DtqnWJob* jobs) {
    DirectPlan p;
    p.n_tiles = direct_tiles(net, jobs, p.dtile0);
    const int per = (p.n_tiles + 7) / 8;
    for (int x = 0; x < 8; ++x) {
        p.xcd_tile0[x] = x * per < p.n_tiles ? x * per : p.n_tiles;
        p.xcd_ntiles[x] = p.n_tiles - p.xcd_tile0[x] < per ? p.n_tiles - p.xcd_tile0[x] : per;
    }
    p.slots = per;
    static_assert(2 * kDSmall / 64 <= kDirectWaves && (size_t)(2 * kDSmall / 64) * kDirectWaves * 64 <= kDirectLdsFloats - kDirectWaves, "small-partial block fits");
    const int n_small = small_elems(net), g1 = p.slots * 8 + (n_small + kDSmall - 1) / kDSmall, g2 = p.slots * 8 + (n_small + 2 * kDSmall - 1) / (2 * kDSmall);
    const int cus = fuse_cu_count();
    p.small_per = (cus > 0 && g1 > cus && g2 <= cus) ? 2 * kDSmall : kDSmall;
    const char* e = getenv("DTQN_DSMALL");
    if (e != nullptr && (atoi(e) == kDSmall || atoi(e) == 2 * kDSmall)) p.small_per = atoi(e);
    p.grid = p.small_per == kDSmall ? g1 : g2;
    p.grid_max = g1;
    return p;
}

}

using namespace dtqn;

extern "C" int dtqn_td_wgrad_splits(const DtqnNet* net, int batch) {
    if (!net || batch < 1) return 1;
    int n = batch < 16 ? batch : 16;
    if (net->n_wjobs <= kMaxWJobs && wgrad_lds_enabled(*net)) {
        DtqnWJob jobs[kMaxWJobs];
        if (dtqn_net_wjobs(net, jobs) == DTQN_OK) {
            int tiles = 0;
            for (int j = 0; j < net->n_wjobs; ++j)
                if (wgrad_lds_job(*net, jobs[j])) tiles += (jobs[j].N / 128) * (jobs[j].K / 128);
            if (tiles > 0) {
                const int cus = device_cu_count() > 0 ? device_cu_count() : 256;
                const char* e = getenv("DTQN_WGRAD_SLOTS");
                const int per_cu = e != nullptr && atoi(e) > 0 ? atoi(e) : 2;
                n = per_cu * cus / tiles;
                n = n < 1 ? 1 : (n > batch ? batch : n);
                n = n > 64 ? 64 : n;
            }
        }
    }
    return n;
}

extern "C" int dtqn_td_wgrad_is_direct(const DtqnNet* net, int batch) {
    if (!net || batch < 1 || net->n_wjobs > kMaxWJobs) return 0;
    if (net->img_c > 0) return 0;
    const char* e = getenv("DTQN_WGRAD_DIRECT");
    if (e != nullptr) return atoi(e) != 0 ? 1 : 0;
    const int gru_layers = net->gate == DTQN_GATE_GRU ? net->num_layers : 1, bag_sets = net->bag_size > 0 ? 2 : 1;
    const int layers = gru_layers > bag_sets ? gru_layers : bag_sets;
    return (long long)batch * net->lp * layers <= kDirectMaxTokens ? 1 : 0;
}

extern "C" int dtqn_td_norm_partials(const DtqnNet* net) {
    if (!net || net->n_wjobs > kMaxWJobs) return 0;
    DtqnWJob jobs[kMaxWJobs];
    if (dtqn_net_wjobs(net, jobs) != DTQN_OK) return 0;
    const int opt = (net->n_trainable + 1023) / 1024, dir = direct_plan(net, jobs).grid_max;
    return opt > dir ? opt : dir;
}

static int wgrad_direct(const DtqnNet* net, const DtqnTd* td, hipStream_t stream) {
    WgradDirectArgs a;
    a.net = *net;
    if (dtqn_net_wjobs(net, a.jobs) != DTQN_OK) return DTQN_ERR_CONFIG;
    for (int j = 0; j < net->n_wjobs; ++j)
        if ((long long)td->batch * net->lp * a.jobs[j].n_layers > kDirectMaxTokens) return DTQN_ERR_CONFIG;
    const DirectPlan plan = direct_plan(net, a.jobs);
    a.n_tiles = plan.n_tiles; a.slots = plan.slots; a.small_per = plan.small_per;
    for (int j = 0; j < net->n_wjobs; ++j) a.dtile0[j] = plan.dtile0[j];
    for (int x = 0; x < 8; ++x) { a.xcd_tile0[x] = plan.xcd_tile0[x]; a.xcd_ntiles[x] = plan.xcd_ntiles[x]; }
    a.act = td->act; a.grd = td->grd; a.grad = td->grad; a.small = td->small;
    a.norm_partial = td->norm_partial; a.step_counter = td->step_counter;
    a.batch = td->batch; a.n_jobs = net->n_wjobs; a.n_small = small_elems(net);
    a.row_split = td->row_split > 1 ? td->row_split : 1;
    a.n_parts = dtqn_td_norm_partials(net);
    const char* xm = getenv("DTQN_WGRAD_XCD");
    a.xcd_map = xm != nullptr ? atoi(xm) : 1;
    const int grid = plan.grid;
    const size_t lds = kDirectLdsFloats * sizeof(float);
    (void)hipGetLastError();
    hipLaunchKernelGGL(dtqn_wgrad_direct_kernel, dim3(grid), dim3(kDirectThreads), lds, stream, a);
    return hipGetLastError() == hipSuccess ? DTQN_OK : DTQN_ERR_LAUNCH;
}

struct WgradLane {
    hipStream_t s;
    hipEvent_t fork, join;
    int state;
};
static WgradLane* wgrad_lane() {
    static WgradLane lanes[kMaxDevices] = {};
    const char* e = getenv("DTQN_WGRAD_SIDE");
    if (e != nullptr && atoi(e) == 0) return nullptr;
    int dev = 0;
    if (hipGetDevice(&dev) != hipSuccess || dev < 0 || dev >= kMaxDevices) return nullptr;
    WgradLane& l = lanes[dev];
    if (l.state == 0) {
        l.state = (hipStreamCreateWithFlags(&l.s, hipStreamNonBlocking) == hipSuccess &&
                   hipEventCreateWithFlags(&l.fork, hipEventDisableTiming) == hipSuccess &&
                   hipEventCreateWithFlags(&l.join, hipEventDisableTiming) == hipSuccess) ? 1 : -1;
        (void)hipGetLastError();
    }
    return l.state == 1 ? &l : nullptr;
}

extern "C" int dtqn_td_wgrad(const DtqnNet* net, const DtqnTd* td, void* stream) {
    if (!net || !td || td->batch < 1 || td->n_split < 1) return DTQN_ERR_ARG;
    if (net->n_wjobs > kMaxWJobs) return DTQN_ERR_CONFIG;
    if (dtqn_td_wgrad_is_fused(net, td)) return DTQN_OK;
    if (dtqn_td_wgrad_is_direct(net, td->batch)) return wgrad_direct(net, td, (hipStream_t)stream);
    WgradArgs a;
    a.net = *net;
    if (dtqn_net_wjobs(net, a.jobs) != DTQN_OK) return DTQN_ERR_CONFIG;
    a.n_jobs = net->n_wjobs;
    a.n_wtiles = net->n_wtiles;
    WgradLdsArgs la;
    bool have_lds = false;
    if (wgrad_lds_enabled(*net)) {
        la.net = *net;
        la.n_jobs = 0; la.n_tiles = 0;
        int keep = 0, tiles = 0;
        for (int j = 0; j < net->n_wjobs; ++j) {
            if (wgrad_lds_job(*net, a.jobs[j])) {
                la.jobs[la.n_jobs].j = a.jobs[j];
                la.jobs[la.n_jobs].tile0 = la.n_tiles;
                la.n_tiles += (a.jobs[j].N / 128) * (a.jobs[j].K / 128);
                ++la.n_jobs;
            } else {
                a.jobs[keep] = a.jobs[j];
                a.jobs[keep].tile0 = tiles;
                tiles += a.jobs[keep].tiles_n * a.jobs[keep].tiles_k;
                ++keep;
            }
        }
        if (la.n_jobs > 0) {
            a.n_jobs = keep; a.n_wtiles = tiles;
            la.act = td->act; la.grd = td->grd; la.gsplit = td->gsplit; la.batch = td->batch; la.n_split = td->n_split;
            have_lds = true;
        }
    }
    WgradLane* lane = have_lds ? wgrad_lane() : nullptr;
    static std::mutex lane_mu;
    std::unique_lock<std::mutex> lk(lane_mu, std::defer_lock);
    hipStream_t small_stream = (hipStream_t)stream;
    if (lane != nullptr) {
        lk.lock();
        if (hipEventRecord(lane->fork, (hipStream_t)stream) == hipSuccess && hipStreamWaitEvent(lane->s, lane->fork, 0) == hipSuccess) small_stream = lane->s;
        else { lane = nullptr; (void)hipGetLastError(); }
    }
    a.act = td->act; a.grd = td->grd; a.gsplit = td->gsplit; a.small = td->small;
    a.batch = td->batch; a.n_split = td->n_split;
    a.row_split = td->row_split > 1 ? td->row_split : 1;
    a.n_small = net->num_layers * 4 * net->d_model + (net->discrete ? net->vocab * net->embed_per_obs : 0) +
                (net->action_dim > 0 ? net->num_actions * net->action_dim : 0) +
                (net->pos == DTQN_POS_LEARNED ? net->ctx_len * net->d_model : 0);
    const int small_blocks = (a.n_small + 1023) / 1024;
    a.small_blocks = small_blocks;
    const char* xm = getenv("DTQN_WGRAD_XCD");
    a.xcd_map = xm != nullptr ? atoi(xm) : 1;
    const int tile_blocks = (a.n_wtiles * td->n_split + 7) / 8 * 8;
    const size_t lds = (size_t)DTQN_WAVES * 65 * 68 * sizeof(float);
    static size_t attr_lds[kMaxDevices] = {};
    raise_lds_limit(reinterpret_cast<const void*>(&dtqn_wgrad_kernel), lds, attr_lds);
    (void)hipGetLastError();
    hipLaunchKernelGGL(dtqn_wgrad_kernel, dim3(tile_blocks + small_blocks * td->n_split), dim3(DTQN_THREADS), lds, small_stream, a);
    if (hipGetLastError() != hipSuccess) return DTQN_ERR_LAUNCH;
    if (lane != nullptr && hipEventRecord(lane->join, lane->s) != hipSuccess) return DTQN_ERR_LAUNCH;
    if (have_lds) {
        const size_t llds = (size_t)kLdsTK * (kLdsLDY + kLdsLDX) * sizeof(float);
        (void)hipGetLastError();
        hipLaunchKernelGGL(dtqn_wgrad_lds_kernel, dim3(la.n_tiles * td->n_split), dim3(kLdsThreads), llds, (hipStream_t)stream, la);
        if (hipGetLastError() != hipSuccess) return DTQN_ERR_LAUNCH;
    }
    if (lane != nullptr && hipStreamWaitEvent((hipStream_t)stream, lane->join, 0) != hipSuccess) return DTQN_ERR_LAUNCH;
    return DTQN_OK;
}
```

### dtqn_amd/csrc/dtqn_wgrad_direct.hpp

```cpp
#pragma once
#include "dtqn_device.hpp"

namespace dtqn {

#ifndef DTQN_DIRECT_WAVES
#define DTQN_DIRECT_WAVES 16
#endif
constexpr int kDirectWaves = DTQN_DIRECT_WAVES;
constexpr int kFuseWaves = 8;
constexpr int kDirectThreads = kDirectWaves * 64;
constexpr int kDirectMaxTokens = 2048;
constexpr int kDTN = 16, kDTK = 32;
constexpr int kDGroup = 8;
#ifndef DTQN_DSMALL
#define DTQN_DSMALL 128
#endif
constexpr int kDSmall = DTQN_DSMALL;
constexpr int kDSmallFused = 256;
constexpr size_t direct_lds_floats(int waves) { return waves + (size_t)waves * (kDTN + 1) * (kDTK + 4); }
constexpr size_t kDirectLdsFloats = direct_lds_floats(kDirectWaves);

struct DirectCtx {
    const float* act;
    const float* grd;
    const float* small;
    float* grad;
    int batch, row_split, n_small;
};

template <bool SC1>
__device__ __forceinline__ float direct_ld(const float* base, const DtqnRsrc& rs, size_t idx) {
    if constexpr (SC1) return dtqn_xch_load1(rs, (int)(idx * 4));
    else return base[idx];
}

template <bool SC1, int WV>
__device__ __forceinline__ float direct_tile(const DtqnNet& net, const DirectCtx& a, const DtqnWJob& job, int local, float* slabs, const Thr& t) {
    const int LP = net.lp, tid = t.tid;
    float ss = 0.f;
    const int tiles_k = (job.K + kDTK - 1) / kDTK;
    const int tiles_n = (job.N + kDTN - 1) / kDTN;
    const bool k_major = tiles_k > tiles_n;
    const int bn = k_major ? local % tiles_n : local / tiles_k, bk = k_major ? local / tiles_n : local - bn * tiles_k;
    const int nbase = bn * kDTN, kbase = bk * kDTK;
    const float* xbase = (job.x_in_act ? a.act : a.grd) + job.x_off;
    const size_t xstride = job.x_in_act ? (size_t)net.act_stride : (size_t)net.grd_stride;
    const size_t ystride = (size_t)net.grd_stride;
    const DtqnRsrc grs = DTQN_XCH_RSRC(a.grd, (size_t)a.batch * net.grd_stride * 4);
    const int ycol = nbase + t.i, xcol = kbase + 2 * t.i;
    const bool yok = ycol < job.ldy, xok = xcol < job.ldx;
    f32x4 acc[2] = {zero4(), zero4()};
    float bsum = 0.f;
    const int nsub = LP / 16;
    const int per_layer = a.batch * nsub, units = per_layer * job.n_layers;
    const int mine = (units - t.wave + WV - 1) / WV;
    constexpr int kMaxGroups = (kDirectMaxTokens / 16 + WV * kDGroup - 1) / (WV * kDGroup);
    constexpr int NBUF = kMaxGroups > 1 ? 2 : 1;
    float av[NBUF][kDGroup][4];
    float2 bv[NBUF][kDGroup][4];
    const int ycol_c = yok ? ycol : 0, xcol_c = xok ? xcol : 0;
    const int wv = __builtin_amdgcn_readfirstlane(t.wave);
    int u_lyr = 0, u_sq = wv / nsub, u_sub = wv - u_sq * nsub, u_m = 0;
    while (u_sq >= a.batch) { u_sq -= a.batch; ++u_lyr; }
    const int inc_sq = WV / nsub, inc_sub = WV - inc_sq * nsub;
    const size_t ylane = (size_t)job.dy_off + (size_t)t.kq * job.ldy + ycol_c;
    const float* xlane = xbase + (size_t)t.kq * job.ldx + xcol_c;
    auto group_load = [&](float (&a4)[kDGroup][4], float2 (&b4)[kDGroup][4]) {
#pragma unroll
        for (int q = 0; q < kDGroup; ++q) {
            const bool live = u_m < mine;
            const int lyr = live ? u_lyr : 0, sq = live ? u_sq : 0, sub = live ? u_sub : 0;
            const size_t yp = ylane + (size_t)sq * ystride + (size_t)lyr * job.dy_lstride + (size_t)(sub * 16) * job.ldy;
            const float* xp = xlane + (size_t)sq * xstride + (size_t)lyr * job.x_lstride + (size_t)(sub * 16) * job.ldx;
#pragma unroll
            for (int k = 0; k < 4; ++k) {
                a4[q][k] = direct_ld<SC1>(a.grd, grs, yp + (size_t)4 * k * job.ldy);
                b4[q][k] = *reinterpret_cast<const float2*>(xp + (size_t)4 * k * job.ldx);
            }
            ++u_m;
            u_sub += inc_sub; u_sq += inc_sq;
            if (u_sub >= nsub) { u_sub -= nsub; ++u_sq; }
            while (u_sq >= a.batch) { u_sq -= a.batch; ++u_lyr; }
        }
    };
    auto group_mma = [&](int g, const float (&a4)[kDGroup][4], const float2 (&b4)[kDGroup][4]) {
#pragma unroll
        for (int q = 0; q < kDGroup; ++q) {
            const float keep = (yok && g * kDGroup + q < mine) ? 1.f : 0.f;
#pragma unroll
            for (int k = 0; k < 4; ++k) {
                const float av_ = keep != 0.f ? a4[q][k] : 0.f;
                bsum += av_;
                acc[0] = mfma16(av_, b4[q][k].x, acc[0]);
                acc[1] = mfma16(av_, b4[q][k].y, acc[1]);
            }
        }
    };
    const int ngroups = (mine + kDGroup - 1) / kDGroup;
    if constexpr (kMaxGroups == 1) {
        group_load(av[0], bv[0]);
        DTQN_SCHED_FENCE();
        group_mma(0, av[0], bv[0]);
    } else {
        constexpr int B1 = NBUF - 1;
        if (ngroups > 0) group_load(av[0], bv[0]);
        DTQN_SCHED_FENCE();
        int g = 0;
        for (; g + 2 < ngroups; g += 2) {
            group_load(av[B1], bv[B1]);
            DTQN_SCHED_FENCE();
            group_mma(g, av[0], bv[0]);
            DTQN_SCHED_FENCE();
            group_load(av[0], bv[0]);
            DTQN_SCHED_FENCE();
            group_mma(g + 1, av[B1], bv[B1]);
            DTQN_SCHED_FENCE();
        }
        if (g + 1 < ngroups) {
            group_load(av[B1], bv[B1]);
            DTQN_SCHED_FENCE();
            group_mma(g, av[0], bv[0]);
            DTQN_SCHED_FENCE();
            group_mma(g + 1, av[B1], bv[B1]);
        } else if (g < ngroups) {
            group_mma(g, av[0], bv[0]);
        }
    }
    bsum += __shfl_xor(bsum, 16);
    bsum += __shfl_xor(bsum, 32);
    constexpr int SLD = kDTK + 4;
    float* slab = slabs + (size_t)t.wave * (kDTN + 1) * SLD;
#pragma unroll
    for (int r = 0; r < 4; ++r)
        *reinterpret_cast<float2*>(slab + (t.kq * 4 + r) * SLD + 2 * t.i) = make_float2(acc[0][r], acc[1][r]);
    if (t.kq == 0) slab[kDTN * SLD + t.i] = bsum;
    __syncthreads();
    if (tid < kDTN * (kDTK / 4)) {
        const int nl = tid / (kDTK / 4), k4 = (tid % (kDTK / 4)) * 4;
        const int n = nbase + nl, k = kbase + k4;
        if (n < job.N && k < job.K) {
            float4 v = ld4(slabs + nl * SLD + k4);
#pragma unroll
            for (int w = 1; w < WV; ++w) {
                const float4 x = ld4(slabs + (size_t)w * (kDTN + 1) * SLD + nl * SLD + k4);
                v.x += x.x; v.y += x.y; v.z += x.z; v.w += x.w;
            }
            float* op = a.grad + job.w_off + (size_t)n * job.K + k;
            if (k + 3 < job.K && (job.K & 3) == 0) {
                st4(op, v);
                ss = (v.x * v.x + v.y * v.y) + (v.z * v.z + v.w * v.w);
            } else {
                const float vv[4] = {v.x, v.y, v.z, v.w};
                for (int c = 0; c < 4; ++c)
                    if (k + c < job.K) { op[c] = vv[c]; ss += vv[c] * vv[c]; }
            }
        }
    } else if (tid >= 256 && tid < 256 + kDTN && job.b_off >= 0 && bk == 0) {
        const int nl = tid - 256, n = nbase + nl;
        if (n < job.N) {
            float v = 0.f;
#pragma unroll
            for (int w = 0; w < WV; ++w) v += slabs[(size_t)w * (kDTN + 1) * SLD + kDTN * SLD + nl];
            a.grad[job.b_off + n] = v;
            ss = v * v;
        }
    }
    return ss;
}

template <bool SC1, int PER, int WV>
__device__ __forceinline__ float direct_small(const DtqnNet& net, const DirectCtx& a, int sb, float* slabs, const Thr& t) {
    constexpr int HN = PER / 64;
    static_assert(HN <= WV, "one finishing wave per 64 elements");
    const int D = net.d_model;
    const int n_ln = net.num_layers * 4 * D;
    const int n_tab = net.discrete ? net.vocab * net.embed_per_obs : 0;
    const int n_act = net.action_dim > 0 ? net.num_actions * net.action_dim : 0;
    const DtqnRsrc grs = DTQN_XCH_RSRC(a.grd, (size_t)a.batch * net.grd_stride * 4);
    const DtqnRsrc srs = DTQN_XCH_RSRC(a.small, (size_t)a.batch * a.row_split * net.sp_parts * net.sp_stride * 4);
    float ss = 0.f;
    int dst[HN];
#pragma unroll
    for (int h = 0; h < HN; ++h) {
        dst[h] = -1;
        const int e = sb * PER + h * 64 + t.lane;
        float v = 0.f;
        if (e < a.n_small) {
            int src;
            bool in_small = true;
            size_t stride = (size_t)net.sp_stride;
            if (e < n_ln) {
                const int l = e / (4 * D);
                dst[h] = net.off_layer0 + l * net.layer_stride + (e - l * 4 * D);
                src = net.so_ln + e;
            } else if (e < n_ln + n_tab) {
                dst[h] = net.off_obs_tab + (e - n_ln);
                src = net.so_tab + (e - n_ln);
            } else if (e < n_ln + n_tab + n_act) {
                dst[h] = net.off_act_emb + (e - n_ln - n_tab);
                src = net.so_act + (e - n_ln - n_tab);
            } else {
                dst[h] = net.off_pos + (e - n_ln - n_tab - n_act);
                src = net.go_dx0 + (e - n_ln - n_tab - n_act);
                in_small = false;
                stride = (size_t)net.grd_stride;
            }
            const int cnt = a.batch * (in_small ? a.row_split * net.sp_parts : 1);
#pragma unroll 8
            for (int q = t.wave; q < cnt; q += WV)
                v += in_small ? direct_ld<SC1>(a.small, srs, (size_t)q * stride + src) : direct_ld<SC1>(a.grd, grs, (size_t)q * stride + src);
        }
        slabs[(h * WV + t.wave) * 64 + t.lane] = v;
    }
    __syncthreads();
    if (t.wave < HN) {
        int d = -1;
#pragma unroll
        for (int h = 0; h < HN; ++h) d = t.wave == h ? dst[h] : d;
        if (d >= 0) {
            float tot = 0.f;
#pragma unroll
            for (int w = 0; w < WV; ++w) tot += slabs[(t.wave * WV + w) * 64 + t.lane];
            a.grad[d] = tot;
            ss = tot * tot;
        }
    }
    return ss;
}

template <int WV>
__device__ __forceinline__ void direct_norm_partial(float ss, float* red, float* norm_partial, int slot, const Thr& t) {
    ss = wave_sum(ss);
    __syncthreads();
    if (t.lane == 0) red[t.wave] = ss;
    __syncthreads();
    if (t.tid == 0) {
        float tot = 0.f;
        for (int w = 0; w < WV; ++w) tot += red[w];
        norm_partial[slot] = tot;
    }
}

inline int direct_tiles_of(const DtqnWJob& j) { return ((j.N + kDTN - 1) / kDTN) * ((j.K + kDTK - 1) / kDTK); }
inline int small_elems(const DtqnNet* net) {
    return net->num_layers * 4 * net->d_model + (net->discrete ? net->vocab * net->embed_per_obs : 0) +
           (net->action_dim > 0 ? net->num_actions * net->action_dim : 0) +
           (net->pos == DTQN_POS_LEARNED ? net->ctx_len * net->d_model : 0);
}

constexpr int kFuseMaxJobs = 16;
constexpr int kFuseMaxEvents = 12;
constexpr int kFuseDeparted = kFuseMaxEvents;
constexpr int kFuseWords = 16;
struct FuseArgs {
    int n_role;
    int n_chain;
    int n_jobs, n_tiles, n_items, n_small, n_parts;
    DtqnWJob jobs[kFuseMaxJobs];
    int dtile0[kFuseMaxJobs];
    int job_event[kFuseMaxJobs];
    float* grad;
    float* norm_partial;
    int32_t* step_counter;
    int32_t* counters;
};

__device__ __forceinline__ void fuse_wait(int32_t* counter, int target, const Thr& t) {
    if (t.tid == 0)
        while (DTQN_AGENT_LOAD(counter) < target) DTQN_SPIN_PAUSE_LONG();
    __syncthreads();
}

template <int NW>
__device__ __forceinline__ void fuse_role(const DtqnNet& net, const FuseArgs& f, const DirectCtx& ctx, int w, float* smem, const Thr& t) {
    static_assert(NW == kFuseWaves, "the weight-gradient workgroups of the backward launch have its eight waves");
    float* red = smem;
    float* slabs = smem + NW;
    float ss = 0.f;
    if (w == 0 && t.tid == 0) f.step_counter[0] = f.step_counter[1];
    if (w == 0)
        for (int i = f.n_role + t.tid; i < f.n_parts; i += NW * 64) f.norm_partial[i] = 0.f;
    const int per_xcd = f.n_role / 8, slot = (w % 8) * per_xcd + w / 8;
    int waited = -1;
#ifndef DTQN_FUSE_DEBUG_PLAINLD
#define DTQN_FUSE_DEBUG_PLAINLD 0
#endif
#ifdef DTQN_FUSE_DEBUG_NOROLE
    for (int p = f.n_items; p < f.n_items; p += f.n_role) {
#else
    for (int p = slot; p < f.n_items; p += f.n_role) {
#endif
        __syncthreads();
        if (p < f.n_tiles) {
            int j = 0;
            for (int k = 1; k < f.n_jobs; ++k)
                if (f.dtile0[k] <= p) j = k;
            const int ev = f.job_event[j];
            if (ev > waited) { fuse_wait(f.counters + ev, f.n_chain, t); waited = ev; }
            ss += direct_tile<!DTQN_FUSE_DEBUG_PLAINLD, NW>(net, ctx, f.jobs[j], p - f.dtile0[j], slabs, t);
        } else {
            if (net.num_layers > waited) { fuse_wait(f.counters + net.num_layers, f.n_chain, t); waited = net.num_layers; }
            ss += direct_small<!DTQN_FUSE_DEBUG_PLAINLD, kDSmallFused, NW>(net, ctx, p - f.n_tiles, slabs, t);
        }
    }
    direct_norm_partial<NW>(ss, red, f.norm_partial, w, t);
    if (net.num_layers > waited) fuse_wait(f.counters + net.num_layers, f.n_chain, t);
    if (t.tid == 0) {
        const int before = DTQN_AGENT_ADD(f.counters + kFuseDeparted, (int32_t)1);
        if (before == f.n_role - 1)
            for (int e = 0; e <= kFuseDeparted; ++e) DTQN_AGENT_STORE(f.counters + e, (int32_t)0);
    }
}

__device__ __forceinline__ void fuse_arrive(int32_t* counters, int e, const Thr& t) {
    if (t.tid == 0) DTQN_AGENT_ADD(counters + e, (int32_t)1);
}

inline int fuse_cu_count() { return device_cu_count(); }
inline bool fuse_plan(const DtqnNet* net, const DtqnTd* td, FuseArgs* f) {
    f->n_role = 0;
    if (!net || !td || td->row_split != 4 || net->tiled || net->gate == DTQN_GATE_GRU || net->identity || net->bag_size > 0 || net->img_c > 0 ||
        dtqn_ws_lite(net->tiled, net->d_model, net->head_dim, net->d_real))
        return false;
    if (!td->grad || !td->norm_partial || !td->step_counter || !td->small || !td->xflags || !td->act || !td->grd) return false;
    if (!dtqn_td_wgrad_is_direct(net, td->batch) || waves_for(*net) != kFuseWaves) return false;
    const int NL = net->num_layers;
    if (net->n_wjobs != 1 + 4 * NL + 2 || net->n_wjobs > kFuseMaxJobs || NL + 1 > kFuseMaxEvents) return false;
    const char* e = getenv("DTQN_WGRAD_FUSED");
    if (e == nullptr || atoi(e) == 0) return false;
    DtqnWJob jobs[kFuseMaxJobs];
    if (dtqn_net_wjobs(net, jobs) != DTQN_OK) return false;
    if (net->grd_stride % 32 != 0 || net->go_dq % 32 != 0 || net->go_dhh % 32 != 0 || net->go_dx0 % 32 != 0 ||
        net->go_layer0 % 32 != 0 || net->grd_layer_stride % 32 != 0 || net->lp % 32 != 0)
        return false;
    for (int j = 0; j < net->n_wjobs; ++j)
        if (!jobs[j].x_in_act) return false;
    const int n_chain = td->batch * 4;
    int n_role = ((fuse_cu_count() - n_chain) / 8) * 8;
    const char* r = getenv("DTQN_FUSE_ROLE_WGS");
    if (r != nullptr) n_role = (atoi(r) / 8) * 8;
    const int n_parts = dtqn_td_norm_partials(net);
    if (n_role > n_parts) n_role = (n_parts / 8) * 8;
    if (n_role < 8) return false;
    int tiles = 0;
    for (int k = 0; k < net->n_wjobs; ++k) {
        const int j = net->n_wjobs - 1 - k;
        f->jobs[k] = jobs[j];
        f->dtile0[k] = tiles;
        tiles += direct_tiles_of(jobs[j]);
        const int layer = j == 0 ? 0 : j > 4 * NL ? NL - 1 : (j - 1) / 4;
        f->job_event[k] = (j == 0 || layer == 0) ? NL : NL - 1 - layer;
    }
    f->n_jobs = net->n_wjobs;
    f->n_tiles = tiles;
    f->n_small = small_elems(net);
    f->n_items = tiles + (f->n_small + kDSmallFused - 1) / kDSmallFused;
    f->n_parts = n_parts;
    f->n_chain = n_chain;
    f->grad = td->grad;
    f->norm_partial = td->norm_partial;
    f->step_counter = td->step_counter;
    f->counters = td->xflags + dtqn_td_xch_flags(net, td->batch) - kFuseWords;
    f->n_role = n_role;
    return true;
}

}
```

Measured before the change: 11510 TD-updates/s.

## Fuse weight-gradient tiles into the target-ahead backward launch's forward blocks

When the backward pass launches together with the next step's target forward, the forward-role workgroups now go on to compute the direct weight-gradient tiles. They wait on per-chain-workgroup flags instead of shared counters, and the separate wgrad launch is skipped through an in-place registry keyed by the gradient pointer. This becomes the default fused mode ('ahead') and uses virtual waves so each workgroup keeps more loads in flight. The intent is to remove a kernel launch and overlap the wgrad work with the backward chain. The cost is spin-waits, more LDS per block, extra flag words, and host-side mutex bookkeeping.

```diff
diff --git a/dtqn_amd/csrc/dtqn_api.cpp b/dtqn_amd/csrc/dtqn_api.cpp
--- a/dtqn_amd/csrc/dtqn_api.cpp
+++ b/dtqn_amd/csrc/dtqn_api.cpp
@@ -20,10 +20,10 @@
 }
 extern "C" void* dtqn_debug_profile_buffer(void) { return g_profile_buffer; }
 
+namespace dtqn { int device_cu_count_cached(); }
 static int policy_cus() {
-    int dev = 0, n = 0;
-    if (hipGetDevice(&dev) != hipSuccess || hipDeviceGetAttribute(&n, hipDeviceAttributeMultiprocessorCount, dev) != hipSuccess || n <= 0) return 256;
-    return n;
+    const int n = dtqn::device_cu_count_cached();
+    return n > 0 ? n : 256;
 }
 extern "C" int dtqn_td_row_split(const DtqnNet* net, int batch) {
     if (!net || batch < 1) return 1;
@@ -65,7 +65,7 @@
 }
 extern "C" int dtqn_td_xch_flags(const DtqnNet* net, int batch) {
     if (!net || batch < 1) return 0;
-    return 3 * batch * net->num_layers * 6 + 16;
+    return 3 * batch * net->num_layers * 6 + (net->num_layers + 1) * 4 * batch + 16;
 }
 
 extern "C" int dtqn_td_update(const DtqnNet* net, const DtqnReplay* rp, const DtqnTd* td, void* stream) {
diff --git a/dtqn_amd/csrc/dtqn_backward.hip b/dtqn_amd/csrc/dtqn_backward.hip
--- a/dtqn_amd/csrc/dtqn_backward.hip
+++ b/dtqn_amd/csrc/dtqn_backward.hip
@@ -1,3 +1,5 @@
+#include <mutex>
+
 #include "dtqn_device.hpp"
 #include "dtqn_bwd_device.hpp"
 #include "dtqn_gru.hpp"
@@ -58,9 +60,18 @@
     static_assert(RS == 1 || RS == 2 || RS == 4, "one, two or four row slices");
     static_assert(!PAD || (RS == 4 && MT == 1 && !GRU && !DROP && !FUSE && D == 64), "width padding rides with the four-slice residual-gate chain");
     if constexpr (AHEAD) {
-        static_assert(RS == 4 && MT == 1 && !GRU && !DROP && !FUSE && D <= 64, "the target pass ahead rides with the four-slice residual-gate chain");
+        static_assert(RS == 4 && MT == 1 && !GRU && !DROP && D <= 64, "the target pass ahead rides with the four-slice residual-gate chain");
         if ((int)blockIdx.x >= a.batch * RS) {
             forward_body_wl<D, 1, HD, NW, 4, false, PAD>(ahead.f);
+            if constexpr (FUSE) {
+                const int w = (int)blockIdx.x - a.batch * RS;
+                if (w < a.fuse.n_role) {
+                    __syncthreads();
+                    DTQN_PROF(a.prof, 0);
+                    const DirectCtx ctx{a.act, a.grd, a.small, a.fuse.grad, a.batch, RS, a.fuse.n_small};
+                    fuse_role_ahead<NW>(a.net, a.fuse, ctx, w, reinterpret_cast<float*>(dtqn_smem), make_thr(), a.prof);
+                }
+            }
             return;
         }
     }
@@ -79,7 +90,7 @@
     const DtqnNet& net = a.net;
     const Thr t = make_thr();
     const Thr& t_outer = t;
-    if constexpr (FUSE) {
+    if constexpr (FUSE && !AHEAD) {
         if ((int)blockIdx.x >= a.batch * RS) {
             const DirectCtx ctx{a.act, a.grd, a.small, a.fuse.grad, a.batch, RS, a.fuse.n_small};
             fuse_role<NW>(net, a.fuse, ctx, (int)blockIdx.x - a.batch * RS, reinterpret_cast<float*>(dtqn_smem), t);
@@ -296,7 +307,7 @@
                 }
                 __syncthreads();
                 if constexpr (FUSE) {
-                    if (c0 == 0 && l + 1 < net.num_layers) fuse_arrive(a.fuse.counters, net.num_layers - 2 - l, t);
+                    if (c0 == 0 && l + 1 < net.num_layers) fuse_arrive(a.fuse, net.num_layers - 2 - l, (int)blockIdx.x, t);
                 }
                 if (SPLITK || DTQN_BWD_GUARD(t.wave, 0)) {
 #pragma unroll
@@ -712,7 +723,7 @@
     if constexpr (FUSE) {
         DTQN_WAIT_VMEM();
         __syncthreads();
-        fuse_arrive(a.fuse.counters, net.num_layers, t);
+        fuse_arrive(a.fuse, net.num_layers, (int)blockIdx.x, t);
     }
 }
 
@@ -739,18 +750,25 @@
     hipLaunchKernelGGL((dtqn_backward_kernel<D, MT, HD, NW, GRU, RS, DROP, FUSE>), dim3(grid), dim3(NW * 64), lds, stream, a, AheadArgs<false>{});
     return hipGetLastError() == hipSuccess ? DTQN_OK : DTQN_ERR_LAUNCH;
 }
-template <int HD, bool PAD = false>
+template <int HD, bool PAD = false, bool FUSE = false>
 static int launch_bwd_ahead(const BwdArgs& a, const FwdArgs& f, hipStream_t stream) {
+    static_assert(sizeof(BwdArgs) + sizeof(AheadArgs<true>) <= 4096, "kernel arguments fit the 4 KB segment");
     const size_t lb = bwd_lds_bytes(&a.net), lf = fwd_lds_bytes(&a.net, true);
-    const size_t lds = lb > lf ? lb : lf;
+    size_t lds = lb > lf ? lb : lf;
+    if constexpr (FUSE) {
+        const size_t lr = (kFuseWaves + direct_lds_floats(kDirectWaves)) * sizeof(float), ls = (kFuseWaves + (size_t)(2 * kDSmall / 64) * kDirectWaves * 64) * sizeof(float);
+        lds = lds > lr ? lds : lr;
+        lds = lds > ls ? lds : ls;
+        if (a.fuse.ahead == 0 || a.fuse.n_role > f.batch * 4 || a.fuse.n_chain != a.batch * 4) return DTQN_ERR_CONFIG;
+    }
     if (lds > 160 * 1024) return DTQN_ERR_CONFIG;
     static size_t attr_lds[kMaxDevices] = {};
-    raise_lds_limit(reinterpret_cast<const void*>(&dtqn_backward_kernel<64, 1, HD, 8, false, 4, false, false, true, PAD>), lds, attr_lds);
+    raise_lds_limit(reinterpret_cast<const void*>(&dtqn_backward_kernel<64, 1, HD, 8, false, 4, false, FUSE, true, PAD>), lds, attr_lds);
     (void)hipGetLastError();
     AheadArgs<true> ah;
     ah.f = f;
     ah.f.block0 = a.batch * 4;
-    hipLaunchKernelGGL((dtqn_backward_kernel<64, 1, HD, 8, false, 4, false, false, true, PAD>), dim3(a.batch * 4 + f.batch * 4), dim3(8 * 64), lds, stream, a, ah);
+    hipLaunchKernelGGL((dtqn_backward_kernel<64, 1, HD, 8, false, 4, false, FUSE, true, PAD>), dim3(a.batch * 4 + f.batch * 4), dim3(8 * 64), lds, stream, a, ah);
     return hipGetLastError() == hipSuccess ? DTQN_OK : DTQN_ERR_LAUNCH;
 }
 template <int HD, bool PAD>
@@ -783,6 +801,35 @@
         else return DTQN_ERR_CONFIG;
     }
     return launch_bwd2<D, MT, HD, NW, false, 1>(a, stream);
+}
+
+int device_cu_count_cached() { return device_cu_count(); }
+
+static std::mutex g_in_place_mu;
+static const float* g_in_place[64] = {};
+bool wgrad_in_place_note(const float* grad, bool in_place) {
+    std::lock_guard<std::mutex> lk(g_in_place_mu);
+    int room = -1;
+    for (int i = 0; i < 64; ++i) {
+        if (g_in_place[i] == grad) {
+            if (!in_place) g_in_place[i] = nullptr;
+            return true;
+        }
+        if (g_in_place[i] == nullptr && room < 0) room = i;
+    }
+    if (!in_place) return true;
+    if (grad == nullptr || room < 0) return false;
+    g_in_place[room] = grad;
+    return true;
+}
+bool wgrad_in_place_take(const float* grad) {
+    std::lock_guard<std::mutex> lk(g_in_place_mu);
+    for (int i = 0; i < 64; ++i)
+        if (grad != nullptr && g_in_place[i] == grad) {
+            g_in_place[i] = nullptr;
+            return true;
+        }
+    return false;
 }
 
 }
@@ -832,7 +879,8 @@
     a.drop_thresh = net->dropout > 0.f ? (uint32_t)((double)net->dropout * 4294967296.0) : 0u;
     a.drop_scale = net->dropout > 0.f ? 1.0f / (1.0f - net->dropout) : 1.0f;
     a.drop_seed = td->dropout_seed; a.step_counter = td->step_counter;
-    fuse_plan(net, td, &a.fuse);
+    if (fuse_plan(net, td, &a.fuse, td_next != nullptr) && td_next != nullptr && !wgrad_in_place_note(td->grad, true)) a.fuse.n_role = a.fuse.ahead = 0;
+    if (a.fuse.ahead == 0) wgrad_in_place_note(td->grad, false);
     const int D = net->d_model, MT = net->lp / 16, HD = net->head_dim, NW = waves_for(*net);
     hipStream_t s = (hipStream_t)stream;
     if (dtqn_ws_lite(net->tiled, D, HD, net->d_real)) {
@@ -869,16 +917,20 @@
             return DTQN_ERR_CONFIG;
         }
         if (td_next != nullptr) {
-            if (td->row_split != 4 || net->gate != DTQN_GATE_RES || a.drop_thresh != 0u || a.fuse.n_role > 0 || !dtqn_td_fwd_slices4_ok(net) ||
-                !td_next->sample_in_kernel || td_next->batch != td->batch || !td_next->xch || !td_next->xflags || !td_next->q3 || NW != 8)
+            if (td->row_split != 4 || net->gate != DTQN_GATE_RES || a.drop_thresh != 0u || (a.fuse.n_role > 0 && !a.fuse.ahead) || !dtqn_td_fwd_slices4_ok(net) ||
+                !td_next->sample_in_kernel || td_next->batch != td->batch || !td_next->xch || !td_next->xflags || !td_next->q3 || NW != 8) {
+                wgrad_in_place_note(td->grad, false);
                 return DTQN_ERR_CONFIG;
+            }
             FwdArgs f;
             td_forward_args(net, rp, td_next, 2, draw_step_next, &f);
             f.nseq = td_next->batch;
             f.prof = nullptr;
-            if (D == 64 && HD == 8) return launch_bwd_ahead<8>(a, f, s);
-            if (D == 64 && HD == 16) return launch_bwd_ahead<16>(a, f, s);
-            return DTQN_ERR_CONFIG;
+            int rc = DTQN_ERR_CONFIG;
+            if (D == 64 && HD == 8) rc = a.fuse.ahead ? launch_bwd_ahead<8, false, true>(a, f, s) : launch_bwd_ahead<8>(a, f, s);
+            else if (D == 64 && HD == 16) rc = a.fuse.ahead ? launch_bwd_ahead<16, false, true>(a, f, s) : launch_bwd_ahead<16>(a, f, s);
+            if (rc != DTQN_OK && a.fuse.ahead) wgrad_in_place_note(td->grad, false);
+            return rc;
         }
         if (td->row_split == 4) {
             if (D == 64 && HD == 8) return launch_bwd2<64, 1, 8, 8, false, 4>(a, s);
diff --git a/dtqn_amd/csrc/dtqn_gfx950.hpp b/dtqn_amd/csrc/dtqn_gfx950.hpp
--- a/dtqn_amd/csrc/dtqn_gfx950.hpp
+++ b/dtqn_amd/csrc/dtqn_gfx950.hpp
@@ -22,6 +22,7 @@
 #define DTQN_SYSTEM_LOAD(p) __hip_atomic_load(p, __ATOMIC_RELAXED, __HIP_MEMORY_SCOPE_SYSTEM)
 #define DTQN_SYSTEM_STORE(p, v) __hip_atomic_store(p, v, __ATOMIC_RELAXED, __HIP_MEMORY_SCOPE_SYSTEM)
 #define DTQN_AGENT_ADD(p, v) __hip_atomic_fetch_add(p, v, __ATOMIC_RELAXED, __HIP_MEMORY_SCOPE_AGENT)
+#define DTQN_AGENT_ACQUIRE() __builtin_amdgcn_fence(__ATOMIC_ACQUIRE, "agent")
 #define DTQN_SPIN_PAUSE() __builtin_amdgcn_s_sleep(2)
 #define DTQN_SPIN_PAUSE_LONG() __builtin_amdgcn_s_sleep(12)
 #define DTQN_WAIT_VMEM() asm volatile("s_waitcnt vmcnt(0)" ::: "memory")
diff --git a/dtqn_amd/csrc/dtqn_wgrad.hip b/dtqn_amd/csrc/dtqn_wgrad.hip
--- a/dtqn_amd/csrc/dtqn_wgrad.hip
+++ b/dtqn_amd/csrc/dtqn_wgrad.hip
@@ -391,10 +391,7 @@
     p.slots = per;
     static_assert(2 * kDSmall / 64 <= kDirectWaves && (size_t)(2 * kDSmall / 64) * kDirectWaves * 64 <= kDirectLdsFloats - kDirectWaves, "small-partial block fits");
     const int n_small = small_elems(net), g1 = p.slots * 8 + (n_small + kDSmall - 1) / kDSmall, g2 = p.slots * 8 + (n_small + 2 * kDSmall - 1) / (2 * kDSmall);
-    const int cus = fuse_cu_count();
-    p.small_per = (cus > 0 && g1 > cus && g2 <= cus) ? 2 * kDSmall : kDSmall;
-    const char* e = getenv("DTQN_DSMALL");
-    if (e != nullptr && (atoi(e) == kDSmall || atoi(e) == 2 * kDSmall)) p.small_per = atoi(e);
+    p.small_per = direct_small_per(p.slots * 8, n_small);
     p.grid = p.small_per == kDSmall ? g1 : g2;
     p.grid_max = g1;
     return p;
@@ -493,6 +490,7 @@
     if (!net || !td || td->batch < 1 || td->n_split < 1) return DTQN_ERR_ARG;
     if (net->n_wjobs > kMaxWJobs) return DTQN_ERR_CONFIG;
     if (dtqn_td_wgrad_is_fused(net, td)) return DTQN_OK;
+    if (wgrad_in_place_take(td->grad)) return DTQN_OK;
     if (dtqn_td_wgrad_is_direct(net, td->batch)) return wgrad_direct(net, td, (hipStream_t)stream);
     WgradArgs a;
     a.net = *net;
diff --git a/dtqn_amd/csrc/dtqn_wgrad_direct.hpp b/dtqn_amd/csrc/dtqn_wgrad_direct.hpp
--- a/dtqn_amd/csrc/dtqn_wgrad_direct.hpp
+++ b/dtqn_amd/csrc/dtqn_wgrad_direct.hpp
@@ -1,4 +1,6 @@
 #pragma once
+#include <cstring>
+
 #include "dtqn_device.hpp"
 
 namespace dtqn {
@@ -34,7 +36,7 @@
     else return base[idx];
 }
 
-template <bool SC1, int WV>
+template <bool SC1, int WV, int VPW = 1>
 __device__ __forceinline__ float direct_tile(const DtqnNet& net, const DirectCtx& a, const DtqnWJob& job, int local, float* slabs, const Thr& t) {
     const int LP = net.lp, tid = t.tid;
     float ss = 0.f;
@@ -49,20 +51,29 @@
     const DtqnRsrc grs = DTQN_XCH_RSRC(a.grd, (size_t)a.batch * net.grd_stride * 4);
     const int ycol = nbase + t.i, xcol = kbase + 2 * t.i;
     const bool yok = ycol < job.ldy, xok = xcol < job.ldx;
-    f32x4 acc[2] = {zero4(), zero4()};
-    float bsum = 0.f;
+    constexpr int VW = WV * VPW;
+    f32x4 acc[VPW][2];
+    float bsum[VPW];
+#pragma unroll
+    for (int v = 0; v < VPW; ++v) { acc[v][0] = zero4(); acc[v][1] = zero4(); bsum[v] = 0.f; }
     const int nsub = LP / 16;
     const int per_layer = a.batch * nsub, units = per_layer * job.n_layers;
-    const int mine = (units - t.wave + WV - 1) / WV;
-    constexpr int kMaxGroups = (kDirectMaxTokens / 16 + WV * kDGroup - 1) / (WV * kDGroup);
-    constexpr int NBUF = kMaxGroups > 1 ? 2 : 1;
+    int mine;
+    constexpr int kMaxGroups = (kDirectMaxTokens / 16 + VW * kDGroup - 1) / (VW * kDGroup);
+    static_assert(VPW == 1 || kMaxGroups == 1, "virtual waves: one group each, all of them in flight at once");
+    constexpr int NBUF = VPW > 1 ? VPW : kMaxGroups > 1 ? 2 : 1;
     float av[NBUF][kDGroup][4];
     float2 bv[NBUF][kDGroup][4];
     const int ycol_c = yok ? ycol : 0, xcol_c = xok ? xcol : 0;
     const int wv = __builtin_amdgcn_readfirstlane(t.wave);
-    int u_lyr = 0, u_sq = wv / nsub, u_sub = wv - u_sq * nsub, u_m = 0;
-    while (u_sq >= a.batch) { u_sq -= a.batch; ++u_lyr; }
-    const int inc_sq = WV / nsub, inc_sub = WV - inc_sq * nsub;
+    int u_lyr, u_sq, u_sub, u_m;
+    auto walk_from = [&](int vw) {
+        mine = (units - vw + VW - 1) / VW;
+        u_lyr = 0; u_sq = vw / nsub; u_sub = vw - u_sq * nsub; u_m = 0;
+        while (u_sq >= a.batch) { u_sq -= a.batch; ++u_lyr; }
+    };
+    walk_from(wv);
+    const int inc_sq = VW / nsub, inc_sub = VW - inc_sq * nsub;
     const size_t ylane = (size_t)job.dy_off + (size_t)t.kq * job.ldy + ycol_c;
     const float* xlane = xbase + (size_t)t.kq * job.ldx + xcol_c;
     auto group_load = [&](float (&a4)[kDGroup][4], float2 (&b4)[kDGroup][4]) {
@@ -83,21 +94,33 @@
             while (u_sq >= a.batch) { u_sq -= a.batch; ++u_lyr; }
         }
     };
-    auto group_mma = [&](int g, const float (&a4)[kDGroup][4], const float2 (&b4)[kDGroup][4]) {
+    auto group_mma = [&](int g, const float (&a4)[kDGroup][4], const float2 (&b4)[kDGroup][4], int v = 0) {
 #pragma unroll
         for (int q = 0; q < kDGroup; ++q) {
             const float keep = (yok && g * kDGroup + q < mine) ? 1.f : 0.f;
 #pragma unroll
             for (int k = 0; k < 4; ++k) {
                 const float av_ = keep != 0.f ? a4[q][k] : 0.f;
-                bsum += av_;
-                acc[0] = mfma16(av_, b4[q][k].x, acc[0]);
-                acc[1] = mfma16(av_, b4[q][k].y, acc[1]);
+                bsum[v] += av_;
+                acc[v][0] = mfma16(av_, b4[q][k].x, acc[v][0]);
+                acc[v][1] = mfma16(av_, b4[q][k].y, acc[v][1]);
             }
         }
     };
     const int ngroups = (mine + kDGroup - 1) / kDGroup;
-    if constexpr (kMaxGroups == 1) {
+    if constexpr (VPW > 1) {
+#pragma unroll
+        for (int v = 0; v < VPW; ++v) {
+            walk_from(wv + v * WV);
+            group_load(av[v], bv[v]);
+        }
+        DTQN_SCHED_FENCE();
+#pragma unroll
+        for (int v = 0; v < VPW; ++v) {
+            mine = (units - (wv + v * WV) + VW - 1) / VW;
+            group_mma(0, av[v], bv[v], v);
+        }
+    } else if constexpr (kMaxGroups == 1) {
         group_load(av[0], bv[0]);
         DTQN_SCHED_FENCE();
         group_mma(0, av[0], bv[0]);
@@ -126,14 +149,17 @@
             group_mma(g, av[0], bv[0]);
         }
     }
-    bsum += __shfl_xor(bsum, 16);
-    bsum += __shfl_xor(bsum, 32);
     constexpr int SLD = kDTK + 4;
-    float* slab = slabs + (size_t)t.wave * (kDTN + 1) * SLD;
-#pragma unroll
-    for (int r = 0; r < 4; ++r)
-        *reinterpret_cast<float2*>(slab + (t.kq * 4 + r) * SLD + 2 * t.i) = make_float2(acc[0][r], acc[1][r]);
-    if (t.kq == 0) slab[kDTN * SLD + t.i] = bsum;
+#pragma unroll
+    for (int v = 0; v < VPW; ++v) {
+        bsum[v] += __shfl_xor(bsum[v], 16);
+        bsum[v] += __shfl_xor(bsum[v], 32);
+        float* slab = slabs + (size_t)(t.wave + v * WV) * (kDTN + 1) * SLD;
+#pragma unroll
+        for (int r = 0; r < 4; ++r)
+            *reinterpret_cast<float2*>(slab + (t.kq * 4 + r) * SLD + 2 * t.i) = make_float2(acc[v][0][r], acc[v][1][r]);
+        if (t.kq == 0) slab[kDTN * SLD + t.i] = bsum[v];
+    }
     __syncthreads();
     if (tid < kDTN * (kDTK / 4)) {
         const int nl = tid / (kDTK / 4), k4 = (tid % (kDTK / 4)) * 4;
@@ -141,7 +167,7 @@
         if (n < job.N && k < job.K) {
             float4 v = ld4(slabs + nl * SLD + k4);
 #pragma unroll
-            for (int w = 1; w < WV; ++w) {
+            for (int w = 1; w < VW; ++w) {
                 const float4 x = ld4(slabs + (size_t)w * (kDTN + 1) * SLD + nl * SLD + k4);
                 v.x += x.x; v.y += x.y; v.z += x.z; v.w += x.w;
             }
@@ -160,7 +186,7 @@
         if (n < job.N) {
             float v = 0.f;
 #pragma unroll
-            for (int w = 0; w < WV; ++w) v += slabs[(size_t)w * (kDTN + 1) * SLD + kDTN * SLD + nl];
+            for (int w = 0; w < VW; ++w) v += slabs[(size_t)w * (kDTN + 1) * SLD + kDTN * SLD + nl];
             a.grad[job.b_off + n] = v;
             ss = v * v;
         }
@@ -168,9 +194,9 @@
     return ss;
 }
 
-template <bool SC1, int PER, int WV>
+template <bool SC1, int PER, int WV, int VPW = 1>
 __device__ __forceinline__ float direct_small(const DtqnNet& net, const DirectCtx& a, int sb, float* slabs, const Thr& t) {
-    constexpr int HN = PER / 64;
+    constexpr int HN = PER / 64, VW = WV * VPW;
     static_assert(HN <= WV, "one finishing wave per 64 elements");
     const int D = net.d_model;
     const int n_ln = net.num_layers * 4 * D;
@@ -184,7 +210,9 @@
     for (int h = 0; h < HN; ++h) {
         dst[h] = -1;
         const int e = sb * PER + h * 64 + t.lane;
-        float v = 0.f;
+        float v[VPW];
+#pragma unroll
+        for (int p = 0; p < VPW; ++p) v[p] = 0.f;
         if (e < a.n_small) {
             int src;
             bool in_small = true;
@@ -206,11 +234,15 @@
                 stride = (size_t)net.grd_stride;
             }
             const int cnt = a.batch * (in_small ? a.row_split * net.sp_parts : 1);
+#pragma unroll
+            for (int p = 0; p < VPW; ++p) {
 #pragma unroll 8
-            for (int q = t.wave; q < cnt; q += WV)
-                v += in_small ? direct_ld<SC1>(a.small, srs, (size_t)q * stride + src) : direct_ld<SC1>(a.grd, grs, (size_t)q * stride + src);
-        }
-        slabs[(h * WV + t.wave) * 64 + t.lane] = v;
+                for (int q = t.wave + p * WV; q < cnt; q += VW)
+                    v[p] += in_small ? direct_ld<SC1>(a.small, srs, (size_t)q * stride + src) : direct_ld<SC1>(a.grd, grs, (size_t)q * stride + src);
+            }
+        }
+#pragma unroll
+        for (int p = 0; p < VPW; ++p) slabs[(h * VW + t.wave + p * WV) * 64 + t.lane] = v[p];
     }
     __syncthreads();
     if (t.wave < HN) {
@@ -220,7 +252,7 @@
         if (d >= 0) {
             float tot = 0.f;
 #pragma unroll
-            for (int w = 0; w < WV; ++w) tot += slabs[(t.wave * WV + w) * 64 + t.lane];
+            for (int w = 0; w < VW; ++w) tot += slabs[(t.wave * VW + w) * 64 + t.lane];
             a.grad[d] = tot;
             ss = tot * tot;
         }
@@ -263,6 +295,11 @@
     float* norm_partial;
     int32_t* step_counter;
     int32_t* counters;
+    int ahead;
+    int32_t* flagw;
+    int otile0[kFuseMaxJobs];
+    int slots, xcd_map, small_per, part_grid;
+    int sc1_loads;
 };
 
 __device__ __forceinline__ void fuse_wait(int32_t* counter, int target, const Thr& t) {
@@ -312,22 +349,119 @@
     }
 }
 
-__device__ __forceinline__ void fuse_arrive(int32_t* counters, int e, const Thr& t) {
-    if (t.tid == 0) DTQN_AGENT_ADD(counters + e, (int32_t)1);
+__device__ __forceinline__ void fuse_arrive(const FuseArgs& f, int e, int chain_wg, const Thr& t) {
+    if (t.tid == 0) {
+        if (f.ahead) DTQN_AGENT_STORE(f.flagw + e * f.n_chain + chain_wg, (int32_t)1);
+        else DTQN_AGENT_ADD(f.counters + e, (int32_t)1);
+    }
+}
+
+#ifndef DTQN_AGENT_ACQUIRE
+#define DTQN_AGENT_ACQUIRE() ((void)0)
+#endif
+__device__ __forceinline__ void fuse_wait_flags(const int32_t* flags, int n, bool acquire, const Thr& t) {
+    if (t.wave == 0) {
+        for (;;) {
+            int miss = 0;
+            for (int i = t.lane; i < n; i += 64) miss |= DTQN_AGENT_LOAD(flags + i) == 0 ? 1 : 0;
+            if (__ballot(miss) == 0ull) break;
+            DTQN_SPIN_PAUSE_LONG();
+        }
+        if (acquire) {
+            DTQN_AGENT_ACQUIRE();
+            DTQN_WAIT_VMEM();
+        }
+    }
+    __syncthreads();
+}
+
+template <int NW>
+__device__ __forceinline__ void fuse_role_ahead(const DtqnNet& net, const FuseArgs& f, const DirectCtx& ctx, int w, float* smem, const Thr& t,
+                                                long long* prof) {
+    static_assert(kDirectWaves % NW == 0, "whole virtual waves per wave");
+    constexpr int VPW = kDirectWaves / NW;
+    float* red = smem;
+    float* slabs = smem + NW;
+    const int NL = net.num_layers, tile_blocks = f.slots * 8;
+    if (w == 0 && t.tid == 0) f.step_counter[0] = f.step_counter[1];
+    if (w == 0)
+        for (int i = t.tid; i < f.n_parts; i += NW * 64) {
+            int left = f.n_tiles - (i % 8) * f.slots;
+            left = left < 0 ? 0 : left > f.slots ? f.slots : left;
+            const bool empty = i >= f.part_grid || (i < tile_blocks && (f.xcd_map ? i / 8 >= left : i >= f.n_tiles));
+            if (empty) f.norm_partial[i] = 0.f;
+        }
+    const int per_xcd = f.n_role / 8, slot = (w % 8) * per_xcd + w / 8;
+    const bool acquire = f.sc1_loads == 0;
+    int waited = -1;
+    for (int p = slot; p < f.n_items; p += f.n_role) {
+        __syncthreads();
+        int j = 0, ev = NL, pslot = tile_blocks + (p - f.n_tiles);
+        if (p < f.n_tiles) {
+            for (int k = 1; k < f.n_jobs; ++k)
+                if (f.dtile0[k] <= p) j = k;
+            ev = f.job_event[j];
+            const int tile = f.otile0[j] + (p - f.dtile0[j]);
+            pslot = f.xcd_map ? (tile % f.slots) * 8 + tile / f.slots : tile;
+        }
+        if (ev > waited) {
+            if (waited >= 0) DTQN_PROF(prof, 2);
+            fuse_wait_flags(f.flagw + ev * f.n_chain, f.n_chain, acquire, t);
+            waited = ev;
+            DTQN_PROF(prof, ev == NL ? 3 : 1);
+        }
+        float ss;
+        if (p < f.n_tiles) {
+            ss = f.sc1_loads ? direct_tile<true, NW, VPW>(net, ctx, f.jobs[j], p - f.dtile0[j], slabs, t)
+                             : direct_tile<false, NW, VPW>(net, ctx, f.jobs[j], p - f.dtile0[j], slabs, t);
+        } else if (f.small_per == 2 * kDSmall) {
+            ss = f.sc1_loads ? direct_small<true, 2 * kDSmall, NW, VPW>(net, ctx, p - f.n_tiles, slabs, t)
+                             : direct_small<false, 2 * kDSmall, NW, VPW>(net, ctx, p - f.n_tiles, slabs, t);
+        } else {
+            ss = f.sc1_loads ? direct_small<true, kDSmall, NW, VPW>(net, ctx, p - f.n_tiles, slabs, t)
+                             : direct_small<false, kDSmall, NW, VPW>(net, ctx, p - f.n_tiles, slabs, t);
+        }
+        direct_norm_partial<NW>(ss, red, f.norm_partial, pslot, t);
+    }
+    DTQN_PROF(prof, 4);
+    if (NL > waited) fuse_wait_flags(f.flagw + NL * f.n_chain, f.n_chain, false, t);
+    int* last = reinterpret_cast<int*>(red);
+    __syncthreads();
+    if (t.tid == 0) *last = DTQN_AGENT_ADD(f.counters + kFuseDeparted, (int32_t)1) == f.n_role - 1 ? 1 : 0;
+    __syncthreads();
+    if (*last) {
+        for (int i = t.tid; i < (NL + 1) * f.n_chain; i += NW * 64) DTQN_AGENT_STORE(f.flagw + i, (int32_t)0);
+        if (t.tid == 0) DTQN_AGENT_STORE(f.counters + kFuseDeparted, (int32_t)0);
+    }
 }
 
 inline int fuse_cu_count() { return device_cu_count(); }
-inline bool fuse_plan(const DtqnNet* net, const DtqnTd* td, FuseArgs* f) {
+enum { kFuseOff = 0, kFuseExtra = 1, kFuseAhead = 2 };
+inline int fuse_mode() {
+    const char* e = getenv("DTQN_WGRAD_FUSED");
+    if (e == nullptr || strcmp(e, "ahead") == 0) return kFuseAhead;
+    return atoi(e) != 0 ? kFuseExtra : kFuseOff;
+}
+inline int direct_small_per(int tile_blocks, int n_small) {
+    const int g1 = tile_blocks + (n_small + kDSmall - 1) / kDSmall, g2 = tile_blocks + (n_small + 2 * kDSmall - 1) / (2 * kDSmall);
+    const int cus = fuse_cu_count();
+    int per = (cus > 0 && g1 > cus && g2 <= cus) ? 2 * kDSmall : kDSmall;
+    const char* e = getenv("DTQN_DSMALL");
+    if (e != nullptr && (atoi(e) == kDSmall || atoi(e) == 2 * kDSmall)) per = atoi(e);
+    return per;
+}
+inline bool fuse_plan(const DtqnNet* net, const DtqnTd* td, FuseArgs* f, bool ahead = false) {
     f->n_role = 0;
+    f->ahead = 0;
+    if (fuse_mode() != (ahead ? kFuseAhead : kFuseExtra)) return false;
     if (!net || !td || td->row_split != 4 || net->tiled || net->gate == DTQN_GATE_GRU || net->identity || net->bag_size > 0 || net->img_c > 0 ||
         dtqn_ws_lite(net->tiled, net->d_model, net->head_dim, net->d_real))
         return false;
+    if (ahead && net->dropout > 0.f) return false;
     if (!td->grad || !td->norm_partial || !td->step_counter || !td->small || !td->xflags || !td->act || !td->grd) return false;
     if (!dtqn_td_wgrad_is_direct(net, td->batch) || waves_for(*net) != kFuseWaves) return false;
     const int NL = net->num_layers;
     if (net->n_wjobs != 1 + 4 * NL + 2 || net->n_wjobs > kFuseMaxJobs || NL + 1 > kFuseMaxEvents) return false;
-    const char* e = getenv("DTQN_WGRAD_FUSED");
-    if (e == nullptr || atoi(e) == 0) return false;
     DtqnWJob jobs[kFuseMaxJobs];
     if (dtqn_net_wjobs(net, jobs) != DTQN_OK) return false;
     if (net->grd_stride % 32 != 0 || net->go_dq % 32 != 0 || net->go_dhh % 32 != 0 || net->go_dx0 % 32 != 0 ||
@@ -336,17 +470,20 @@
     for (int j = 0; j < net->n_wjobs; ++j)
         if (!jobs[j].x_in_act) return false;
     const int n_chain = td->batch * 4;
-    int n_role = ((fuse_cu_count() - n_chain) / 8) * 8;
+    int n_role = ahead ? (n_chain / 8) * 8 : ((fuse_cu_count() - n_chain) / 8) * 8;
     const char* r = getenv("DTQN_FUSE_ROLE_WGS");
-    if (r != nullptr) n_role = (atoi(r) / 8) * 8;
+    if (r != nullptr && !ahead) n_role = (atoi(r) / 8) * 8;
     const int n_parts = dtqn_td_norm_partials(net);
-    if (n_role > n_parts) n_role = (n_parts / 8) * 8;
+    if (n_role > n_parts && !ahead) n_role = (n_parts / 8) * 8;
     if (n_role < 8) return false;
+    int otile0[kFuseMaxJobs], otiles = 0;
+    for (int j = 0; j < net->n_wjobs; ++j) { otile0[j] = otiles; otiles += direct_tiles_of(jobs[j]); }
     int tiles = 0;
     for (int k = 0; k < net->n_wjobs; ++k) {
         const int j = net->n_wjobs - 1 - k;
         f->jobs[k] = jobs[j];
         f->dtile0[k] = tiles;
+        f->otile0[k] = otile0[j];
         tiles += direct_tiles_of(jobs[j]);
         const int layer = j == 0 ? 0 : j > 4 * NL ? NL - 1 : (j - 1) / 4;
         f->job_event[k] = (j == 0 || layer == 0) ? NL : NL - 1 - layer;
@@ -354,15 +491,27 @@
     f->n_jobs = net->n_wjobs;
     f->n_tiles = tiles;
     f->n_small = small_elems(net);
-    f->n_items = tiles + (f->n_small + kDSmallFused - 1) / kDSmallFused;
+    f->slots = (tiles + 7) / 8;
+    f->small_per = ahead ? direct_small_per(f->slots * 8, f->n_small) : kDSmallFused;
+    f->n_items = tiles + (f->n_small + f->small_per - 1) / f->small_per;
+    f->part_grid = f->slots * 8 + (f->n_small + f->small_per - 1) / f->small_per;
+    const char* xm = getenv("DTQN_WGRAD_XCD");
+    f->xcd_map = xm != nullptr ? atoi(xm) : 1;
+    const char* sl = getenv("DTQN_FUSE_SC1LD");
+    f->sc1_loads = sl != nullptr && atoi(sl) != 0 ? 1 : 0;
+    f->ahead = ahead ? 1 : 0;
     f->n_parts = n_parts;
     f->n_chain = n_chain;
     f->grad = td->grad;
     f->norm_partial = td->norm_partial;
     f->step_counter = td->step_counter;
     f->counters = td->xflags + dtqn_td_xch_flags(net, td->batch) - kFuseWords;
+    f->flagw = f->counters - (NL + 1) * n_chain;
     f->n_role = n_role;
     return true;
 }
 
-}
+bool wgrad_in_place_note(const float* grad, bool in_place);
+bool wgrad_in_place_take(const float* grad);
+
+}
```

After: 10760 TD-updates/s. 0.934x the previous value.
